# vasudeva-ram/Julia-NewtonRaphsonHANK

Hardware: AMD Instinct MI355X
Metric: sequence-space JVPs/sec (household block: BackwardIteration+ForwardIteration+aggregation, Krusell-Smith T=300) (higher is better)
Workload: dtype f64; 1 GPU; ks_2000x11_T300_N32; grid=2000x11, T=300, tangents_per_gpu=32, step=1 dual-sweep pass: primal + N tangents (hank_primal_jvp), parallelism=tangent-sharded x1

## Files before the change

julia-newtonraphsonhank_amd/csrc/hank_device.h:

```cpp
#pragma once
#include <hip/hip_runtime.h>
#include <stdint.h>
#include "hank_geom.h"

#ifndef HANK_XFWD_LQ
#define HANK_XFWD_LQ 1
#endif
#ifndef HANK_XFWD_EARLY_BATCH
#define HANK_XFWD_EARLY_BATCH 0
#endif

namespace hank {

struct Consts {
    int n_a, n_e, G, P;
    int n_hh;
    int diet;
    double beta, gamma, bc;
    const double *a, *z, *Pi;
};

struct Record {
    double *s, *kc, *A, *B, *u, *v, *pol, *lw, *ig, *Dseq;
    int *ib, *lo, *start, *clo;
    int4 *seg;
    double2 *lwg;
};

__device__ inline double wave_sum(double x) {
#pragma unroll
    for (int off = 32; off > 0; off >>= 1) x += __shfl_down(x, off, 64);
    return x;
}
__device__ inline double block_sum(double x, double *red, int nthreads) {
    const int lane = threadIdx.x & 63, wv = threadIdx.x >> 6;
    const int nw = (nthreads + 63) >> 6;
    x = wave_sum(x);
    __syncthreads();
    if (lane == 0) red[wv] = x;
    __syncthreads();
    double r = 0.0;
    if (threadIdx.x == 0)
        for (int k = 0; k < nw; k++) r += red[k];
    return r;
}

__device__ __forceinline__ void lds_barrier() { asm volatile("s_waitcnt lgkmcnt(0)\n\ts_barrier" ::: "memory"); }

__device__ __forceinline__ void st_wt(double *p, double x) {
    __hip_atomic_store(reinterpret_cast<unsigned long long *>(p), (unsigned long long)__double_as_longlong(x), __ATOMIC_RELAXED, __HIP_MEMORY_SCOPE_AGENT);
}

__device__ __forceinline__ double mix_mul(double p, double v) { return p * v; }
__device__ __forceinline__ double2 mix_mul(double p, double2 v) { return make_double2(p * v.x, p * v.y); }
__device__ __forceinline__ double mix_add(double a, double b) { return a + b; }
__device__ __forceinline__ double2 mix_add(double2 a, double2 b) { return make_double2(a.x + b.x, a.y + b.y); }
template <typename T>
__device__ __forceinline__ T mix_sum(T acc, const T *V, int vs, const double *P, int ps, int k0, int n) {
    int k = k0;
    for (; k + 3 < n; k += 4) {
        const T v0 = V[k * vs], v1 = V[(k + 1) * vs], v2 = V[(k + 2) * vs], v3 = V[(k + 3) * vs];
        const double p0 = P[k * ps], p1 = P[(k + 1) * ps], p2 = P[(k + 2) * ps], p3 = P[(k + 3) * ps];
// ... 411 lines not shown
    lds_barrier();
    if constexpr (NX > 0) {
#pragma unroll
        for (int o = 0; o < NX; o++) sh[o][e * 64 + lane] = vadd(partx[o], paggx[o]);
        lds_barrier();
        if (e == 0) {
#pragma unroll
            for (int o = 0; o < NX; o++) {
                VT s = sh[o][lane];
                for (int k = 1; k < c.n_e; k++) s = vadd(s, sh[o][k * 64 + lane]);
                for (int off = 32; off >= g.NC; off >>= 1) s = vadd(s, vshfl_xor(s, off));
                if (rl == 0 && nok) hx.parts[(((size_t)t * nbx_total + bidx) * NX + o) * N + n] = s;
            }
        }
    }
    if (e == 0) {
        VT s = red[lane], s2 = red2[lane];
        for (int k = 1; k < c.n_e; k++) { s = vadd(s, red[k * 64 + lane]); s2 = vadd(s2, red2[k * 64 + lane]); }
        for (int off = 32; off >= g.NC; off >>= 1) { s = vadd(s, vshfl_xor(s, off)); s2 = vadd(s2, vshfl_xor(s2, off)); }
        if (rl == 0 && nok) {
            aggpart[((size_t)t * nbx_total + bidx) * 2 * N + n] = s;
            aggpart[((size_t)t * nbx_total + bidx) * 2 * N + N + n] = s2;
        }
    }
}

constexpr int HX_NS = 5;

constexpr int ADJ_KS = 3;

template <typename VT>
__device__ __forceinline__ VT adj_rows_sum(VT v, int NC) {
    for (int off = 32; off >= NC; off >>= 1) v = vadd(v, vshfl_xor(v, off));
    return v;
}

template <typename VT, int NX>
struct AdjHx { const double *f, *fc; const VT *ybx; };
template <typename VT>
struct AdjHx<VT, 0> {};

struct SsCtl { int stop, iters; double resid; };

enum { ERR_KNOTS = 3, ERR_DOMAIN = 4, ERR_NONMONO = 6 };

__device__ inline void set_err(int *err, int code, int t, int e, int j) {
    if (atomicCAS(&err[0], 0, code) == 0) {
        err[1] = t;
        err[2] = e;
        err[3] = j;
    }
}

__device__ __forceinline__ void lottery_body(const Consts &c, const Record &R, int col, int *err, int write_seg, int use_ib, int *shlo, int *sh_clo, int4 *lq = nullptr) {
    const int t = col / c.n_e, e = col % c.n_e;
    const size_t base = (size_t)col * c.n_a;
    const int n = c.n_a;
    if (threadIdx.x == 0) *sh_clo = 0;
    __syncthreads();
    for (int j = threadIdx.x; j < n; j += blockDim.x) {
        const double p = R.pol[base + j];
        int lo = -1, hi = n;
        if (use_ib) {
            const int g0 = min(max(R.ib[base + j], 0), n - 2);
            const double a0 = c.a[g0], a1 = c.a[g0 + 1];
            if (a0 < p && p <= a1) { lo = g0; hi = g0 + 1; }
            else if (g0 > 0 && p <= a0 && c.a[g0 - 1] < p) { lo = g0 - 1; hi = g0; }
        }
        while (hi - lo > 1) {
            const int mid = lo + ((hi - lo) >> 1);
            if (c.a[mid] < p) lo = mid; else hi = mid;
        }
        int l;
        double w, ig;
        if (hi == 0) {
            l = 0; w = 0.0; ig = 0.0;
            atomicMax(sh_clo, j + 1);
        } else if (hi >= n) {
            l = n - 2; w = 1.0; ig = 0.0;
        } else {
            l = hi - 1;
            const double gap = c.a[hi] - c.a[l];
            w = (p - c.a[l]) / gap;
            ig = 1.0 / gap;
        }
        R.lo[base + j] = l; R.lw[base + j] = w; R.ig[base + j] = ig;
        if (lq) lq[base + j] = make_int4(__double2loint(w), __double2hiint(w), l, (hi == 0 || hi >= n) ? 1 : 0);
        shlo[j] = (hi == 0) ? -1 : l;
    }
    __syncthreads();
    const int clo = *sh_clo;
    if (threadIdx.x == 0) R.clo[col] = clo;
    int *st = R.start + (size_t)col * (n + 1);
    int *shst = shlo + n;
    for (int j = threadIdx.x; j < n; j += blockDim.x) {
        const int prev = j ? shlo[j - 1] : -1, cur = shlo[j];
        if (cur < prev) set_err(err, ERR_NONMONO, t, e, j);
        for (int r = (prev < 0 ? 0 : prev + 1); r <= cur; r++) shst[r] = j;
        if (j == n - 1)
            for (int r = (cur < 0 ? 0 : cur + 1); r <= n; r++) shst[r] = n;
    }
    __syncthreads();
    for (int r = threadIdx.x; r <= n; r += blockDim.x) st[r] = shst[r];
    if (write_seg)
        for (int r = threadIdx.x; r < n; r += blockDim.x)
            R.seg[base + r] = make_int4(r > 0 ? shst[r - 1] : shst[r], shst[r], shst[r + 1], 0);
}

struct AdjLane { int e, nl, rl, RB, m; bool mok; };
__device__ __forceinline__ AdjLane adj_lane(const AdjGeom &g) {
    AdjLane L;
    const int lane = threadIdx.x & 63;
    L.e = __builtin_amdgcn_readfirstlane((int)(threadIdx.x >> 6));
    L.nl = lane & (g.NC - 1); L.rl = lane >> g.lgNC; L.RB = 64 >> g.lgNC;
    L.m = blockIdx.y * g.NC + L.nl;
    L.mok = L.m < g.MV;
    return L;
}

template <typename VT, typename Load, typename Begin, typename Src>
__device__ __forceinline__ void adj_dist_body(const Consts &c, const Record &R, const AdjGeom &g, const AdjLane &L, int t, double *adj_sh, Load load,
                                              Begin begin, Src src) {
    const int NS = g.R + 2, n = c.n_a, ne = c.n_e;
    VT *tile = reinterpret_cast<VT *>(adj_sh);
    double *Pish = adj_sh + (size_t)ne * NS * g.NC * (sizeof(VT) / sizeof(double));
    const int e = L.e, nl = L.nl, rl = L.rl, RB = L.RB;
    const int r0 = blockIdx.x * g.R, r1 = min(r0 + g.R, n);
    for (int k = threadIdx.x; k < ne * ne; k += 64 * ne) Pish[k] = c.Pi[k];
#pragma unroll
    for (int k = 0; k < ADJ_KS; k++) {
        const int slot = rl + k * RB;
        if (slot < NS) {
            const int row = slot == g.R + 1 ? 0 : r0 + slot;
            VT v;
            vzero(v);
            if (L.mok && row <= r1 && row < n) v = load(row);
            tile[((size_t)e * NS + slot) * g.NC + nl] = v;
        }
    }
// ... 134 lines not shown
```

julia-newtonraphsonhank_amd/csrc/hank_hip.hip:

```cpp
#include "hank_kernels.h"
#include "hank_xsweep.h"
#include "hank_xspec.h"
#include "hank_jacobian.h"
#include "hank_wide.h"
#include "hank_hetx.h"
#include "hank_scen.h"
#include "hank_ssbatch.h"
#include "hank_adjoint.h"
#include "hank_boundary.h"
#include "hank_ssdiff_launch.h"
#include "../../include/hank_hip.h"

#include <cstdarg>
#include <cstdio>
#include <cstdlib>
#include <cstring>
#include <initializer_list>
#include <list>
#include <mutex>
#include <new>
#include <vector>

using namespace hank;

// ... 156 lines not shown
    void destroy() { for (One &o : s) { if (o.ev0) (void)hipEventDestroy(o.ev0); if (o.ev1) (void)hipEventDestroy(o.ev1); } }
    hipError_t begin(Span k, hipStream_t st) { s[k].valid = false; s[k].from = s[k].ev0; return hipEventRecord(s[k].ev0, st); }
    hipError_t end(Span k, hipStream_t st, int launches) { const hipError_t e = hipEventRecord(s[k].ev1, st); s[k].launches = launches; s[k].valid = e == hipSuccess; return e; }
    hipError_t end_begin(Span k, int launches, Span next, hipStream_t st) { s[next].valid = false; s[next].from = s[k].ev1; return end(k, st, launches); }
    void invalidate(std::initializer_list<Span> ks) { for (Span k : ks) s[k].valid = false; }
    void absent(Span k, int launches) { s[k].valid = false; s[k].launches = launches; }
    hipError_t read(Span k, double *ms, int32_t *launches) const {
        float f = -1.f;
        const hipError_t e = s[k].valid ? hipEventElapsedTime(&f, s[k].from, s[k].ev1) : hipSuccess;
        *ms = e == hipSuccess ? f : -1.0;
        if (launches) *launches = s[k].launches;
        return e;
    }
};
enum Stat { SWEEP_LAUNCHES, TANGENT_WORKSPACES_ALLOCATED, GRAPHS_CAPTURED, SCHEDULE, FALLBACKS, VFI_ITERATIONS, PRIMAL_MEMO_HITS, PRIMAL_SWEEPS, N_STATS };

struct hank_ctx {
    int device = 0;
    Consts c{};
    Record R{};
    int T = 0;
    DevBuf<double> d_a, d_z, d_Pi;
    DevBuf<double> d_ss_value;
    double *d_ss_D = nullptr;
    DevBuf<double> d_xhh, d_agg, d_aggpart;
    DevBuf<double> d_agg_rm;
    DevBuf<double> d_zd;
    DevBuf<int> d_err;
    int nbp = 0;
    bool boundary_set = false, primal_done = false;
    hipStream_t own_stream = nullptr, stream = nullptr;
    hipStream_t side_stream = nullptr;
    hipEvent_t ev_fork = nullptr, ev_side = nullptr;
    bool side_pending = false;
    GraphExec g_pback, g_pfwd;
    Spans spans;
    std::list<TanWork> tws;
    int schedule = 2;
    bool forced_xcd = false;
    TanBatch batch;
    int xjvp_max = 64;
    XWork xw;
    struct { DevBuf<double> dpT, iota, E, Cp, F, Dv, W, dsum; int N = 0, n_het = 0; } fn;
    int wide_mode = 0, wide_min = 80, num_cus = 256, wide_r = 2;
    size_t lds_max = 65536;
    DevBuf<char> rec_slab;
    size_t rec_bytes = 0;
    int4 *rec_lq = nullptr;
    double *rec_iga = nullptr;
    DevBuf<int> d_ibw;
    bool seg_valid = true;
    bool lwg_valid = true;
    long long lwg_builds = 0;
    bool wprep_valid = false;
    std::list<WTan> wtans;
    std::list<CotWork> cws;
    CotBatch cot;
    DevBuf<int> d_adj_sb;
    bool adj_seg_valid = false;
    DevBuf<double> d_bnd_q;
    HxRecord hx;
    ScenWork scen;
    int scen_pending = 0;
    std::vector<double> h_Pi, h_z;
    long long stats[N_STATS] = {};
    bool memo_on = true;
    bool xdual_back = true;
    bool memo_valid = false;
    std::vector<double> memo_xhh;
    int n_het = 2;
    DevBuf<char> hx_slab;
    size_t hx_bytes = 0;
    bool stationary = false;
    std::vector<double> h_ss_value, h_ss_D;
    hipEvent_t ev_stream = nullptr;
    char errmsg[512] = {0};
};

static int fail(hank_ctx *ctx, int code, const char *fmt, ...);
static int het_max(const hank_ctx *ctx) { return ctx->c.n_hh > 2 ? 4 : 3; }
static int hx_count(const hank_ctx *ctx) { return het_max(ctx) - 2; }
static void batch_none(hank_ctx *ctx) { ctx->batch.current = false; ctx->batch.ws = nullptr; }
static void cot_none(hank_ctx *ctx) { ctx->cot = CotBatch(); }
static void cot_ran(hank_ctx *ctx, const void *ws, int M, const double *pbar) { ctx->cot = CotBatch{true, M, ws, pbar}; }
static void batch_ran(hank_ctx *ctx, int family, const void *ws, int N, const double *dagg_cm, const double *dpol, const std::vector<XPass> *passes = nullptr) {
    ctx->batch = TanBatch{family, true, N, ws, dagg_cm, dpol, passes};
}
static void batch_ran_boundary(hank_ctx *ctx, const void *ws, int N, const double *dagg_cm, const double *dpol, const double *zm) {
    batch_ran(ctx, 0, ws, N, dagg_cm, dpol);
    ctx->batch.boundary = true;
    ctx->batch.bnd_zm = zm;
}
static int batch_current(hank_ctx *ctx, int N, const TanBatch **out) {
    if (!ctx->batch.current || ctx->batch.N != N) return fail(ctx, HANK_ERR_NOT_READY, "no tangent sweep with N=%d is current", N);
    *out = &ctx->batch;
    return HANK_OK;
}
static void record_rewritten(hank_ctx *ctx, bool seg_written, bool lwg_written) {
    ctx->primal_done = true; ctx->seg_valid = seg_written; ctx->lwg_valid = lwg_written;
    ctx->wprep_valid = false; ctx->xw.src_valid = false; ctx->xw.rng_valid = false; ctx->adj_seg_valid = false; ctx->hx.valid = false;
    batch_none(ctx);
    cot_none(ctx);
}
static void record_gone(hank_ctx *ctx) {
    record_rewritten(ctx, false, false);
    ctx->primal_done = false;
}
static hipError_t join_side(hank_ctx *ctx) {
    if (!ctx->side_pending) return hipSuccess;
    ctx->side_pending = false;
    return hipStreamWaitEvent(ctx->stream, ctx->ev_side, 0);
}

static int fail(hank_ctx *ctx, int code, const char *fmt, ...) {
    if (ctx) {
        va_list ap;
        va_start(ap, fmt);
        vsnprintf(ctx->errmsg, sizeof(ctx->errmsg), fmt, ap);
        va_end(ap);
    }
    return code;
}

static int het_count_ok(hank_ctx *ctx, const char *who, int n_het, bool declared, bool rest_ok = true) {
    const int max_het = het_max(ctx);
    if (n_het < 1 || n_het > max_het || !rest_ok)
        return fail(ctx, HANK_ERR_BAD_ARG, "%s: bad argument: n_het must be 1..%d (the policy variable, consumption, Value%s), got %d", who, max_het, max_het > 3 ? ", UCE" : "", n_het);
    if (declared && n_het > ctx->n_het)
        return fail(ctx, HANK_ERR_NOT_READY, "%s: %d outputs asked for, %d declared: call hank_set_het_outputs first", who, n_het, ctx->n_het);
    return HANK_OK;
}

static int hip_status(hipError_t e) {
    if (e == hipErrorOutOfMemory) return HANK_ERR_NOMEM;
    if (e == hipErrorNoDevice || e == hipErrorInvalidDevice || e == hipErrorNotInitialized || e == hipErrorInsufficientDriver) return HANK_ERR_NO_DEVICE;
    return HANK_ERR_LAUNCH;
}
#define HIPC(ctx, call)                                                                         \
    do {                                                                                        \
        hipError_t e_ = (call);                                                                 \
        if (e_ != hipSuccess)                                                                   \
            return fail(ctx, hip_status(e_),                                                   \
                        "HIP error %d (%s) at %s:%d: %s", (int)e_, hipGetErrorString(e_),       \
                        __FILE__, __LINE__, #call);                                             \
    } while (0)

struct DeviceGuard {
    int prev = -1;
    bool switched = false, ok = true;
    explicit DeviceGuard(const hank_ctx *ctx);
    ~DeviceGuard() { if (switched) (void)hipSetDevice(prev); }
};
DeviceGuard::DeviceGuard(const hank_ctx *ctx) {
    if (!ctx) return;
    if (hipGetDevice(&prev) != hipSuccess) { ok = false; return; }
    if (prev != ctx->device) { switched = hipSetDevice(ctx->device) == hipSuccess; ok = switched; }
}
#define ENTER(ctx)                                                                                                       \
// ... 450 lines not shown
        w.passes.push_back(ps);
    }
    if ((int)w.passes.size() > XPASS_MAX) return fail(ctx, HANK_ERR_BAD_ARG, "N=%d needs %d passes, at most %d per call", N, (int)w.passes.size(), XPASS_MAX);
    HIPC(ctx, w.dxhh.alloc((size_t)c.n_hh * P * N));
    HIPC(ctx, w.dxr.alloc(P * N)); HIPC(ctx, w.dxw.alloc(P * N)); HIPC(ctx, w.dxt.alloc(P * N));
    HIPC(ctx, w.dpol.alloc(off));
    const size_t W = (size_t)XG * X.dmax, nb = (size_t)X.Sact;
    HIPC(ctx, w.daggpart.alloc(2 * P * nb * W));
    HIPC(ctx, hipMemsetAsync(w.daggpart, 0, sizeof(double) * 2 * P * nb * W, ctx->stream));
    HIPC(ctx, w.dagg_pass.alloc(2 * P * W));
    HIPC(ctx, w.dagg_cm.alloc(2 * P * N));
    return HANK_OK;
}
static int x_ensure_tan(hank_ctx *ctx, int N, XTan **out) {
    const int nmax = 8 * ctx->xw.dmax * XPASS_MAX;
    if (N > nmax) return fail(ctx, HANK_ERR_BAD_ARG, "N=%d exceeds %d directions per call", N, nmax);
    return tan_cache_get(ctx, ctx->xw.tans, N, [ctx](XTan &w) { return x_build_tan(ctx, w); }, out);
}

static dim3 x_block(const XWork &X, const Consts &c) {
    const bool fits = 64 * (c.n_e + 1) <= X.maxt && X.syncwave;
    return dim3(fits ? 64 * (c.n_e + 1) : 64 * c.n_e);
}

template <typename F>
static void x_by_maxt(const XWork &X, F launch) { if (X.maxt == 768) launch(std::integral_constant<int, 768>()); else launch(std::integral_constant<int, 1024>()); }
#define XL(...) hipLaunchKernelGGL((__VA_ARGS__), dim3(X.grid), x_block(X, c), lds, sec.stream(), a)
static bool x_has_dual_back(const XWork &X) { return X.maxt == 768; }
static void x_launch_dual_back(XSection &sec, XWork &X, const Consts &c, int D, const XDualBackArgs &a) {
    const size_t lds = x_lds_dual_back(c, D);
    if (!x_has_dual_back(X)) return;
    const XSpec sp = x_spec(X.xspec, c.n_e, c.gamma, c.diet);
    X.inst[0] = sp.ne; X.inst[1] = sp.crra;
    if (!sp.ne && !sp.crra) {
        if (D == 1) XL(k_xdual_back<1, 768>);
        else if (D == 2) XL(k_xdual_back<2, 768>);
        else XL(k_xdual_back<4, 768>);
        return;
    }
    auto by_d = [&](auto ne, auto crra) {
        constexpr int NE = decltype(ne)::value, CRRA = decltype(crra)::value;
        if (D == 1) XL(k_xdual_back<1, 768, NE, CRRA>);
        else if (D == 2) XL(k_xdual_back<2, 768, NE, CRRA>);
        else XL(k_xdual_back<4, 768, NE, CRRA>);
    };
    auto by_crra = [&](auto ne) {
        if (sp.crra) by_d(ne, std::integral_constant<int, 1>()); else if constexpr (decltype(ne)::value != 0) by_d(ne, std::integral_constant<int, 0>());
    };
    if (sp.ne == 4) by_crra(std::integral_constant<int, 4>());
    else if (sp.ne == 7) by_crra(std::integral_constant<int, 7>());
    else if (sp.ne == 11) by_crra(std::integral_constant<int, 11>());
    else by_crra(std::integral_constant<int, 0>());
}
static void x_launch_fwd(XSection &sec, XWork &X, const Consts &c, int D, bool val, const XSweepFwdArgs &a) {
    if (val && D > 0) { X.inst[2] = 0; X.inst[3] = 0; }
#if HANK_XFWD_LQ
    if (val && D > 0 && x_lds_fwd_lq(c, D) <= (size_t)X.lds_max) {
        const size_t lds = x_lds_fwd_lq(c, D);
        x_by_maxt(X, [&](auto mt) {
            constexpr int MT = decltype(mt)::value;
            if (D == 1) XL(k_xfwd<1, true, MT, true>);
            else if (D == 2) XL(k_xfwd<2, true, MT, true>);
            else if (D == 4) { if constexpr (MT == 768) XL(k_xfwd<4, true, MT, true>); }
        });
        return;
    }
#endif
    const size_t lds = x_lds_fwd(c, D, val || D == 0);
    x_by_maxt(X, [&](auto mt) {
        constexpr int MT = decltype(mt)::value;
        if (D == 0) XL(k_xfwd<0, true, MT>);
        else if (D == 1) { if (val) XL(k_xfwd<1, true, MT>); else XL(k_xfwd<1, false, MT>); }
        else if (D == 2) { if (val) XL(k_xfwd<2, true, MT>); else XL(k_xfwd<2, false, MT>); }
        else if (D == 4) { if constexpr (MT == 768) { if (val) XL(k_xfwd<4, true, MT>); else XL(k_xfwd<4, false, MT>); } }
    });
}
static void x_launch_primal_back(XSection &sec, const XWork &X, const Consts &c, const XBackArgs &a) { const size_t lds = x_lds_primal_back(c); x_by_maxt(X, [&](auto mt) { XL(k_xprimal_back<decltype(mt)::value>); }); }
static void x_launch_tan_back(XSection &sec, const XWork &X, const Consts &c, int D, const XTanBackArgs &a) {
    const size_t lds = x_lds_tan_back(c, D);
    x_by_maxt(X, [&](auto mt) {
        constexpr int MT = decltype(mt)::value;
        if (D == 1) XL(k_xtan_back<1, MT>);
        else if (D == 2) XL(k_xtan_back<2, MT>);
        else if (D == 4) { if constexpr (MT == 768) XL(k_xtan_back<4, MT>); }
    });
}
static void x_ensure_rng(XSection &sec) {
    hank_ctx *ctx = sec.ctx;
    XWork &X = ctx->xw;
    if (X.rng_valid) return;
    hipLaunchKernelGGL(k_xunits_fwd, dim3((unsigned)ctx->c.P, (unsigned)X.Sact), dim3(256), 0, sec.stream(), ctx->c, ctx->R, X.Sact, X.srcF, X.unitsF, X.unit_overflow, X.ucap);
    X.rng_valid = true;
}

static int ensure_seg(hank_ctx *ctx) {
    if (ctx->seg_valid) return HANK_OK;
    hipLaunchKernelGGL(k_seg_build, dim3((unsigned)(ctx->c.P * ctx->c.n_e)), dim3(256), 0, ctx->stream, ctx->c, ctx->R, ctx->c.P * ctx->c.n_e);
    HIPC(ctx, hipGetLastError());
    ctx->seg_valid = true;
    return HANK_OK;
}
static int ensure_lwg(hank_ctx *ctx) {
    if (ctx->lwg_valid) return HANK_OK;
    const XWork &X = ctx->xw;
    hipLaunchKernelGGL(k_xlwg_build, dim3((unsigned)(ctx->c.P * ctx->c.n_e)), dim3(256), 0, ctx->stream, ctx->c, ctx->R, X.Dvirt, X.D0own, X.Sact);
    HIPC(ctx, hipGetLastError());
    ctx->lwg_valid = true;
    ctx->lwg_builds++;
    return HANK_OK;
}
static int x_sync_reset(XSection &sec, XSync *base, int count, int where) {
    hank_ctx *ctx = sec.ctx;
    HIPC(ctx, hipMemsetAsync(base, 0, sizeof(XSync) * (size_t)count, sec.stream()));
    if (ctx->xw.fault && ctx->xw.fault != 3 && (ctx->xw.fault_where & where)) hipLaunchKernelGGL(k_xpoison, dim3(1), dim3(64), 0, sec.stream(), base, count, (unsigned)ctx->xw.fault);
    return HANK_OK;
}

static void x_rho(XSection &sec) {
    hank_ctx *ctx = sec.ctx;
    hipLaunchKernelGGL(k_xrho, dim3((unsigned)((ctx->c.P + 255) / 256)), dim3(256), 0, sec.stream(), ctx->d_xhh, ctx->c.n_hh, ctx->c.P, ctx->xw.rho);
}
static void x_tan_in(XSection &sec, XTan *w) {
    const Consts &c = sec.ctx->c;
    hipLaunchKernelGGL(k_tan_in, dim3((unsigned)(((size_t)c.P * w->N + 255) / 256)), dim3(256), 0, sec.stream(), w->dxhh, c.n_hh, c.P, w->N, w->dxr, w->dxw, w->dxt);
}
static int x_tan_front(XSection &sec, XTan *w) {
    hank_ctx *ctx = sec.ctx; XWork &X = ctx->xw;
    const int rc = x_sync_reset(sec, X.sync + 2, 2 * (int)w->passes.size(), 2); if (rc) return rc;
    x_tan_in(sec, w);
    x_rho(sec);
    if (!X.src_valid) {
        hipLaunchKernelGGL(k_xsrc_back, dim3((unsigned)ctx->c.P, X.Sact), dim3(256), 0, sec.stream(), ctx->c, ctx->R, X.Sact, X.srcB);
        X.src_valid = true;
    }
    return HANK_OK;
}
static XRecOff x_rec_off(const hank_ctx *ctx) {
    const Record &R = ctx->R;
    const char *b = ctx->rec_slab;
    auto off = [&](const void *p) { return (unsigned)((const char *)p - b); };
    XRecOff o{};
    o.rec = b; o.bytes = (unsigned)ctx->rec_bytes;
    o.pol = off(R.pol); o.ib = off(R.ib); o.A = off(R.A); o.B = off(R.B); o.u = off(R.u); o.v = off(R.v); o.s = off(R.s); o.kc = off(R.kc);
    o.lo = off(R.lo); o.lw = off(R.lw); o.ig = off(R.ig); o.Dseq = off(R.Dseq);
    o.lq = ctx->rec_lq ? off(ctx->rec_lq) : 0u;
    return o;
}
static bool x_dual_addr_fits(const hank_ctx *ctx) {
    const Consts &c = ctx->c;
    return x_addr_fits(ctx->rec_bytes, (unsigned long long)c.P, XG, (unsigned long long)c.G, XD_MAX, (unsigned long long)((c.n_a + XRW - 1) / XRW), XUCAP);
}
static int x_back(XSection &sec, XTan *dual = nullptr) {
    hank_ctx *ctx = sec.ctx; XWork &X = ctx->xw;
    const Consts &c = ctx->c;
    XBackArgs ab{};
    ab.c = c; ab.ss_value = ctx->d_ss_value; ab.xhh = ctx->d_xhh; ab.rho = X.rho; ab.sy = X.sync; ab.st_s = X.st_s;
// ... 16 lines not shown
#if HANK_XFWD_LQ
    if (lq) {
        hipLaunchKernelGGL(k_lottery_lq, dim3((unsigned)(c.P * c.n_e)), dim3(256), sizeof(int) * (2 * (size_t)c.n_a + 2), sec.stream(), c, ctx->R, c.P * c.n_e, ctx->d_err, seg ? 1 : 0, 1, ctx->rec_lq);
        return;
    }
#endif
    hipLaunchKernelGGL(k_lottery, dim3((unsigned)(c.P * c.n_e)), dim3(256), sizeof(int) * (2 * (size_t)c.n_a + 2), sec.stream(), c, ctx->R, c.P * c.n_e, ctx->d_err, seg ? 1 : 0, 1);
}
static int x_tan_back(XSection &sec, XTan *w) {
    hank_ctx *ctx = sec.ctx; XWork &X = ctx->xw;
    const int np = (int)w->passes.size();
    XTanBackArgs ab{};
    ab.c = ctx->c; ab.R = ctx->R; ab.rho = X.rho; ab.xhh = ctx->d_xhh; ab.dxr = w->dxr; ab.dxw = w->dxw; ab.dxt = w->dxt; ab.Ntot = w->N; ab.st_ds = X.st_ds;
    ab.src = X.neigh ? X.srcB.get() : nullptr;
    ab.stall = X.fault == 3 ? 1 : 0;
    HIPC(ctx, ctx->spans.begin(TAN_BACK, sec.stream()));
    for (int p = 0; p < np; p++) {
        const XPass &ps = w->passes[p];
        ab.n0 = ps.n0; ab.N = ps.N; ab.groups = ps.groups; ab.sy = X.sync + 2 + 2 * p; ab.dpol = w->dpol + ps.dpol_off;
        x_launch_tan_back(sec, X, ctx->c, ps.D, ab);
    }
    HIPC(ctx, ctx->spans.end(TAN_BACK, sec.stream(), np));
    return HANK_OK;
}
static void x_value_epilogue(XSection &sec) {
    hank_ctx *ctx = sec.ctx; const XWork &X = ctx->xw;
    const Consts &c = ctx->c;
    const size_t P = c.P;
    hipStream_t s = sec.stream();
    hipLaunchKernelGGL(k_reduce_parts, dim3((unsigned)P, 1), dim3(256), 0, s, X.aggpart, X.Sact, 2, ctx->d_agg_rm);
    hipLaunchKernelGGL(k_tan_out, dim3((unsigned)((2 * P + 255) / 256)), dim3(256), 0, s, ctx->d_agg_rm, (int)P, 2, ctx->d_agg);
    hipLaunchKernelGGL(k_xfix_D, dim3((unsigned)((P * c.n_e + 255) / 256)), dim3(256), 0, s, c, ctx->R.Dseq, X.Dvirt, X.Sact, X.D0own);
}
static XSweepFwdArgs x_fwd_args(const hank_ctx *ctx, bool val) {
    const XWork &X = ctx->xw;
    XSweepFwdArgs fa{};
    fa.c = ctx->c; fa.R = ctx->R; fa.src = X.srcF; fa.units = X.unitsF; fa.overflow = X.unit_overflow; fa.all_members = X.neigh ? 0 : 1;
    if (val) { fa.D0 = ctx->d_ss_D; fa.Dvirt = X.Dvirt; fa.aggpart = X.aggpart; }
    return fa;
}
static int x_fwd_value(XSection &sec) {
    hank_ctx *ctx = sec.ctx; XWork &X = ctx->xw;
    XSweepFwdArgs fa = x_fwd_args(ctx, true);
    fa.sy = X.sync + 1; fa.st = X.st_D; fa.groups = 1;
    HIPC(ctx, ctx->spans.begin(PRIMAL_FWD, sec.stream()));
    x_launch_fwd(sec, X, ctx->c, 0, true, fa);
    HIPC(ctx, ctx->spans.end(PRIMAL_FWD, sec.stream(), 1));
    x_value_epilogue(sec);
    return HANK_OK;
}
static int x_tan_fwd(XSection &sec, XTan *w, int p, bool val) {
    hank_ctx *ctx = sec.ctx; XWork &X = ctx->xw;
    const XPass &ps = w->passes[p];
    if (!val) { const int rc = ensure_lwg(ctx); if (rc) return rc; }
    XSweepFwdArgs fa = x_fwd_args(ctx, val);
    fa.sy = X.sync + 2 + 2 * p + 1; fa.st = X.st_dD; fa.daggpart = w->daggpart; fa.groups = ps.groups; fa.dpol = w->dpol + ps.dpol_off;
    fa.ro = x_rec_off(ctx); fa.dpol_bytes = (unsigned)((size_t)ctx->c.P * ps.groups * ctx->c.G * ps.D * sizeof(double));
    fa.iga = ctx->rec_iga ? (unsigned)((const char *)ctx->rec_iga - (const char *)ctx->rec_slab) : 0u;
    x_launch_fwd(sec, X, ctx->c, ps.D, val, fa);
    return HANK_OK;
}
static void x_tan_reduce(XSection &sec, XTan *w, int p) {
    hank_ctx *ctx = sec.ctx;
    const size_t P = ctx->c.P;
    const XPass &ps = w->passes[p];
    const int W = XG * ps.D;
    hipStream_t s = sec.stream();
    hipLaunchKernelGGL(k_reduce_parts, dim3((unsigned)P, (2 * W + 63) / 64), dim3(256), 0, s, w->daggpart, ctx->xw.Sact, 2 * W, w->dagg_pass);
    hipLaunchKernelGGL(k_xout, dim3((unsigned)((P * ps.N + 255) / 256)), dim3(256), 0, s, w->dagg_pass, (int)P, 2 * W, 0, ps.n0, ps.N, w->dagg_cm);
    hipLaunchKernelGGL(k_xout, dim3((unsigned)((P * ps.N + 255) / 256)), dim3(256), 0, s, w->dagg_pass, (int)P, 2 * W, W, ps.n0, ps.N, w->dagg_cm + P * (size_t)w->N);
}
static int x_tan_fwd_from(XSection &sec, XTan *w, int first) {
    hank_ctx *ctx = sec.ctx;
    const int np = (int)w->passes.size();
    for (int p = first; p < np; p++) {
        const int rc = x_tan_fwd(sec, w, p, false); if (rc) return rc;
        if (p == np - 1) HIPC(ctx, ctx->spans.end(TAN_FWD, sec.stream(), np));
        x_tan_reduce(sec, w, p);
    }
    return HANK_OK;
}
static void x_dual_epilogue(XSection &sec, XTan *w, double *d_agg_out, double *d_dagg_out) {
    hank_ctx *ctx = sec.ctx; const XWork &X = ctx->xw;
    const Consts &c = ctx->c;
    const XPass &ps = w->passes[0];
    const int W = XG * ps.D, per = 2 * W + 2 + c.n_e;
    hipLaunchKernelGGL(k_xdual_epilogue, dim3((unsigned)(((size_t)c.P * per + 255) / 256)), dim3(256), 0, sec.stream(), c, X.aggpart, w->daggpart, X.Sact, W, ps.n0, ps.N, w->N,
                       ctx->d_agg_rm, ctx->d_agg, w->dagg_pass, w->dagg_cm, ctx->R.Dseq, X.Dvirt, X.D0own, d_agg_out, d_dagg_out);
}

static int x_status(hank_ctx *ctx, const char *what, const XSync *fetched) {
    XWork &X = ctx->xw;
    std::vector<XSync> own;
    if (!fetched) {
        if (!X.ready || X.last_blocks == 0) return HANK_OK;
        int uo = 0;
        HIPC(ctx, hipMemcpy(&uo, X.unit_overflow, sizeof(int), hipMemcpyDeviceToHost));
        if (uo) {
            HIPC(ctx, hipMemsetAsync(X.unit_overflow, 0, sizeof(int), ctx->stream));
            return fail(ctx, HANK_ERR_SWEEP, "persistent forward sweep: a member's walk over its sources needs more than %d work units (a savings policy this flat is served by the per-period launches)", XUCAP);
        }
        own.resize((size_t)X.last_blocks);
        HIPC(ctx, hipMemcpy(own.data(), X.sync, sizeof(XSync) * own.size(), hipMemcpyDeviceToHost));
    }
    const XSync *h = fetched ? fetched : own.data();
    for (size_t k = 0; k < (fetched ? 1 : own.size()); k++)
// ... 328 lines not shown
        return HANK_OK;
    }
    HIPC(ctx, join_side(ctx));
    HIPC(ctx, hipMemcpyAsync(ctx->d_ss_value, ss_end_value, sizeof(double) * G, hipMemcpyHostToDevice, ctx->stream));
    HIPC(ctx, hipMemcpyAsync(ctx->d_ss_D, ss_init_D, sizeof(double) * G, hipMemcpyHostToDevice, ctx->stream));
    {
        const int ne = ctx->c.n_e, na = ctx->c.n_a, P = ctx->c.P;
        std::vector<double> m(ne, 0.0), m2(ne), zd(2 * (size_t)P);
        for (int e = 0; e < ne; e++) for (int i = 0; i < na; i++) m[e] += ss_init_D[(size_t)e * na + i];
        for (int t = 0; t < P; t++) {
            for (int e2 = 0; e2 < ne; e2++) { double v = 0.0; for (int e = 0; e < ne; e++) v += ctx->h_Pi[e + (size_t)ne * e2] * m[e]; m2[e2] = v; }
            m.swap(m2);
            double z = 0.0, one = 0.0;
            for (int e = 0; e < ne; e++) { z += ctx->h_z[e] * m[e]; one += m[e]; }
            zd[t] = z; zd[(size_t)P + t] = one;
        }
        HIPC(ctx, hipMemcpyAsync(ctx->d_zd, zd.data(), sizeof(double) * 2 * P, hipMemcpyHostToDevice, ctx->stream));
    }
    HIPC(ctx, hipStreamSynchronize(ctx->stream));
    ctx->boundary_set = true;
    record_gone(ctx);
    ctx->memo_valid = false;
    ctx->stationary = false;
    ctx->h_ss_value.assign(ss_end_value, ss_end_value + G);
    ctx->h_ss_D.assign(ss_init_D, ss_init_D + G);
    ctx->errmsg[0] = 0;
    return HANK_OK;
}

static void note_primal_x(hank_ctx *ctx, const double *xhh) {
    const size_t n = (size_t)ctx->c.n_hh * ctx->c.P, nh = ctx->c.n_hh;
    if (!xhh) { ctx->memo_valid = false; ctx->stationary = false; return; }
    ctx->memo_xhh.assign(xhh, xhh + n);
    ctx->memo_valid = true;
    bool constant = true;
    for (size_t k = nh; k < n && constant; k++) constant = xhh[k] == xhh[k - nh];
    ctx->stationary = constant;
}

static int run_primal(hank_ctx *ctx, double *d_agg_out) {
    HIPC(ctx, join_side(ctx));
    HIPC(ctx, ctx->spans.begin(PRIMAL_BACK, ctx->stream));
    HIPC(ctx, hipGraphLaunch(ctx->g_pback, ctx->stream));
    HIPC(ctx, ctx->spans.end(PRIMAL_BACK, ctx->stream, ctx->c.P + 2));
    HIPC(ctx, hipEventRecord(ctx->ev_fork, ctx->stream));
    HIPC(ctx, hipStreamWaitEvent(ctx->side_stream, ctx->ev_fork, 0));
    HIPC(ctx, ctx->spans.begin(PRIMAL_FWD, ctx->side_stream));
    HIPC(ctx, hipGraphLaunch(ctx->g_pfwd, ctx->side_stream));
    HIPC(ctx, ctx->spans.end(PRIMAL_FWD, ctx->side_stream, ctx->c.P + 1));
    HIPC(ctx, copy_agg(ctx, d_agg_out, hipMemcpyDeviceToDevice, ctx->side_stream));
    HIPC(ctx, hipEventRecord(ctx->ev_side, ctx->side_stream));
    ctx->side_pending = true;
    ctx->spans.invalidate({DUAL_BACK, DUAL_FWD});
    record_rewritten(ctx, true, true);
    return HANK_OK;
}

static int x_primal(hank_ctx *ctx, const double *xhh, hipMemcpyKind kind, double *d_agg_out) {
    int rc = x_setup(ctx); if (rc) return rc;
    HIPC(ctx, hipMemcpyAsync(ctx->d_xhh, xhh, sizeof(double) * ctx->c.n_hh * ctx->c.P, kind, ctx->stream));
    XSection sec(ctx);
    HIPC(ctx, sec.opened());
    rc = x_sync_reset(sec, ctx->xw.sync, 2, 1); if (rc) return rc;
    zero_err(ctx, sec.stream());
    x_rho(sec);
    rc = x_back(sec); if (rc) return rc;
    x_lottery(sec, true);
    record_rewritten(ctx, true, true);
    x_ensure_rng(sec);
    rc = x_fwd_value(sec); if (rc) return rc;
    HIPC(ctx, hipGetLastError());
    HIPC(ctx, sec.close());
    ctx->stats[SWEEP_LAUNCHES] += 2;
    ctx->xw.last_blocks = 2;
    ctx->spans.invalidate({TAN_BACK, TAN_FWD, DUAL_BACK, DUAL_FWD});
    HIPC(ctx, copy_agg(ctx, d_agg_out, hipMemcpyDeviceToDevice, ctx->stream));
    return HANK_OK;
}
static int x_jvp(hank_ctx *ctx, const double *dxhh, hipMemcpyKind kind, int N, double *d_dagg_out) {
    int rc = x_setup(ctx); if (rc) return rc;
    XTan *w = nullptr;
    rc = x_ensure_tan(ctx, N, &w); if (rc) return rc;
    const int np = (int)w->passes.size();
    HIPC(ctx, hipMemcpyAsync(w->dxhh, dxhh, sizeof(double) * ctx->c.n_hh * ctx->c.P * N, kind, ctx->stream));
    XSection sec(ctx);
    HIPC(ctx, sec.opened());
    rc = x_tan_front(sec, w); if (rc) return rc;
    x_ensure_rng(sec);
    rc = x_tan_back(sec, w); if (rc) return rc;
    HIPC(ctx, ctx->spans.begin(TAN_FWD, sec.stream()));
    rc = x_tan_fwd_from(sec, w, 0); if (rc) return rc;
    HIPC(ctx, hipGetLastError());
    HIPC(ctx, sec.close());
    ctx->stats[SWEEP_LAUNCHES] += 2 * np;
    ctx->xw.last_blocks = 2 + 2 * np;
    ctx->spans.invalidate({DUAL_BACK, DUAL_FWD});
    batch_ran(ctx, 1, w, N, w->dagg_cm, w->dpol, &w->passes);
    HIPC(ctx, copy_dagg(ctx, d_dagg_out, w->dagg_cm, N, hipMemcpyDeviceToDevice));
    return HANK_OK;
}
static void x_dual_ran(hank_ctx *ctx, XTan *w, int launches) {
    ctx->stats[SWEEP_LAUNCHES] += launches;
    ctx->xw.last_blocks = 2 + 2 * (int)w->passes.size();
    ctx->spans.absent(PRIMAL_FWD, 1);
    ctx->spans.invalidate({DUAL_BACK, DUAL_FWD});
    batch_ran(ctx, 1, w, w->N, w->dagg_cm, w->dpol, &w->passes);
}
static int x_dual_two(hank_ctx *ctx, XTan *w, const double *xhh, const double *dxhh, hipMemcpyKind kind, double *d_agg_out, double *d_dagg_out) {
    const size_t nP = (size_t)ctx->c.n_hh * ctx->c.P;
    const int np = (int)w->passes.size();
    XSection sec(ctx);
    HIPC(ctx, sec.opened());
    HIPC(ctx, hipMemcpyAsync(w->dxhh, dxhh, sizeof(double) * nP * w->N, kind, sec.stream()));
    HIPC(ctx, hipMemcpyAsync(ctx->d_xhh, xhh, sizeof(double) * nP, kind, sec.stream()));
    int rc = x_sync_reset(sec, ctx->xw.sync, 2, 1); if (rc) return rc;
    zero_err(ctx, sec.stream());
    x_rho(sec);
    rc = x_back(sec); if (rc) return rc;
    x_lottery(sec, true, true);
    record_rewritten(ctx, true, false);
    x_ensure_rng(sec);
    rc = x_tan_front(sec, w);
    if (!rc) rc = x_tan_back(sec, w);
    if (rc) return rc;
    HIPC(ctx, ctx->spans.begin(TAN_FWD, sec.stream()));
    rc = x_tan_fwd(sec, w, 0, true); if (rc) return rc;
    if (np == 1) {
        HIPC(ctx, ctx->spans.end(TAN_FWD, sec.stream(), 1));
        x_dual_epilogue(sec, w, d_agg_out, d_dagg_out);
    } else {
        x_value_epilogue(sec);
        x_tan_reduce(sec, w, 0);
        rc = x_tan_fwd_from(sec, w, 1); if (rc) return rc;
    }
    HIPC(ctx, hipGetLastError());
    HIPC(ctx, sec.close());
    x_dual_ran(ctx, w, 1 + 2 * np);
    if (np > 1) {
        HIPC(ctx, copy_agg(ctx, d_agg_out, hipMemcpyDeviceToDevice, ctx->stream));
        HIPC(ctx, copy_dagg(ctx, d_dagg_out, w->dagg_cm, w->N, hipMemcpyDeviceToDevice));
    }
    return HANK_OK;
}
static int x_dual_fused(hank_ctx *ctx, XTan *w, const double *xhh, const double *dxhh, hipMemcpyKind kind, bool prologue, double *d_agg_out, double *d_dagg_out) {
    XWork &X = ctx->xw;
    const size_t nP = (size_t)ctx->c.n_hh * ctx->c.P;
    XSection sec(ctx);
    HIPC(ctx, sec.opened());
    if (prologue) {
        hipLaunchKernelGGL(k_xdual_prologue, dim3(64), dim3(256), 0, sec.stream(), xhh, ctx->d_xhh, dxhh, w->dxhh, ctx->c.n_hh, ctx->c.P, w->N, X.rho, w->dxr, w->dxw, w->dxt,
                           reinterpret_cast<xv4u *>(X.sync.get()), sizeof(XSync) * 4 / sizeof(xv4u), ctx->d_err);
    } else {
        HIPC(ctx, hipMemcpyAsync(w->dxhh, dxhh, sizeof(double) * nP * w->N, kind, sec.stream()));
        HIPC(ctx, hipMemcpyAsync(ctx->d_xhh, xhh, sizeof(double) * nP, kind, sec.stream()));
        int rc = x_sync_reset(sec, X.sync, 2, 1);
        if (!rc) rc = x_sync_reset(sec, X.sync + 2, 2, 2);
        if (rc) return rc;
        zero_err(ctx, sec.stream());
        x_rho(sec);
        x_tan_in(sec, w);
    }
    int rc = x_back(sec, w); if (rc) return rc;
    x_lottery(sec, false, true);
    record_rewritten(ctx, false, false);
    x_ensure_rng(sec);
    HIPC(ctx, ctx->spans.begin(TAN_BACK, sec.stream()));
    HIPC(ctx, ctx->spans.end(TAN_BACK, sec.stream(), 1));
    HIPC(ctx, ctx->spans.begin(TAN_FWD, sec.stream()));
    rc = x_tan_fwd(sec, w, 0, true); if (rc) return rc;
    HIPC(ctx, ctx->spans.end(TAN_FWD, sec.stream(), 1));
    x_dual_epilogue(sec, w, d_agg_out, d_dagg_out);
    HIPC(ctx, hipGetLastError());
    HIPC(ctx, sec.close());
    x_dual_ran(ctx, w, 2);
    return HANK_OK;
}
static bool x_dual_back_fits(const hank_ctx *ctx, int D);
static int x_dual(hank_ctx *ctx, const double *xhh, const double *dxhh, hipMemcpyKind kind, int N, double *d_agg_out, double *d_dagg_out) {
    int rc = x_setup(ctx); if (rc) return rc;
    XTan *w = nullptr;
    rc = x_ensure_tan(ctx, N, &w); if (rc) return rc;
    if (w->passes.size() != 1 || !x_dual_back_fits(ctx, w->passes[0].D)) return x_dual_two(ctx, w, xhh, dxhh, kind, d_agg_out, d_dagg_out);
    return x_dual_fused(ctx, w, xhh, dxhh, kind, kind == hipMemcpyDeviceToDevice && !ctx->xw.fault, d_agg_out, d_dagg_out);
}
static bool use_x_primal(const hank_ctx *ctx) { return ctx->schedule >= 1; }
static bool x_tan_fits(const hank_ctx *ctx, int N) {
    const XWork &X = ctx->xw;
    int D = 1;
    while (XG * D < N && D < X.dmax) D *= 2;
    return std::max(x_lds_tan_back(ctx->c, D), x_lds_fwd(ctx->c, D, true)) <= (size_t)X.lds_max;
}
static bool use_x_jvp(const hank_ctx *ctx, int N) { return (ctx->schedule == 1 || (ctx->schedule == 2 && N <= ctx->xjvp_max)) && x_tan_fits(ctx, N); }
static bool x_dual_back_fits(const hank_ctx *ctx, int D) {
    const XWork &X = ctx->xw;
    return ctx->xdual_back && x_has_dual_back(X) && 64 * (ctx->c.n_e + 1) <= X.maxt && x_lds_dual_back(ctx->c, D) <= (size_t)X.lds_max;
}
static bool use_x_fused(const hank_ctx *ctx, int N) {
    if (ctx->schedule < 1 || !x_tan_fits(ctx, N) || !x_dual_addr_fits(ctx)) return false;
    if (ctx->schedule == 1) return true;
    return N <= XG * ctx->xw.dmax && x_dual_back_fits(ctx, ctx->xw.dmax);
}

static int check_rates(hank_ctx *ctx, const double *xhh) {
    for (int t = 0; t < ctx->c.P; t++)
        if (!(1.0 + xhh[ctx->c.n_hh * t] > 0.0)) return fail(ctx, HANK_ERR_DOMAIN, "1 + r must be positive (period %zu)", (size_t)t + 1);
    return HANK_OK;
}
static int enqueue_primal(hank_ctx *ctx, const double *xhh, hipMemcpyKind kind, double *d_agg_out) {
    if (use_x_primal(ctx)) return x_primal(ctx, xhh, kind, d_agg_out);
    HIPC(ctx, hipMemcpyAsync(ctx->d_xhh, xhh, sizeof(double) * ctx->c.n_hh * ctx->c.P, kind, ctx->stream));
    return run_primal(ctx, d_agg_out);
}

int hank_primal_dev(hank_ctx *ctx, const double *d_xhh, double *d_agg_out) {
    ENTER(ctx);
    if (!ctx || !d_xhh) return fail(ctx, HANK_ERR_BAD_ARG, "null pointer");
    if (!ctx->boundary_set) return fail(ctx, HANK_ERR_NOT_READY, "hank_set_boundary must be called first");
    note_primal_x(ctx, nullptr);
    ctx->stats[PRIMAL_SWEEPS]++;
    return enqueue_primal(ctx, d_xhh, hipMemcpyDeviceToDevice, d_agg_out);
}

int hank_check(hank_ctx *ctx) {
    ENTER(ctx);
    if (!ctx) return HANK_ERR_BAD_ARG;
    bool moved = false;
    const int rc = fallback_decision(ctx, device_verdict(ctx, THE_RECORD), &moved);
    return rc ? rc : scen_pending_verdict(ctx);
}

int hank_primal(hank_ctx *ctx, const double *xhh, double *agg_out) {
    ENTER(ctx);
    if (!ctx || !xhh) return fail(ctx, HANK_ERR_BAD_ARG, "null pointer");
    if (!ctx->boundary_set) return fail(ctx, HANK_ERR_NOT_READY, "hank_set_boundary must be called first");
    { const int rrc = check_rates(ctx, xhh); if (rrc) return rrc; }
    note_primal_x(ctx, nullptr);
    const int rc = run_settled(ctx, [&] { return enqueue_primal(ctx, xhh, hipMemcpyHostToDevice, nullptr); });
    if (rc) return rc;
    if (agg_out) {
        HIPC(ctx, copy_agg(ctx, agg_out, hipMemcpyDeviceToHost, ctx->stream));
        HIPC(ctx, hipStreamSynchronize(ctx->stream));
    }
    note_primal_x(ctx, xhh);
    ctx->stats[PRIMAL_SWEEPS]++;
    ctx->errmsg[0] = 0;
    return HANK_OK;
}

static int run_jvp(hank_ctx *ctx, TanWork &w, bool bnd, bool zm, int NX) {
    const int grc = ensure_tan_graphs(ctx, w, bnd, NX);
    if (grc) return grc;
    HIPC(ctx, ctx->spans.begin(TAN_BACK, ctx->stream));
    HIPC(ctx, hipGraphLaunch(w.tan_back(bnd), ctx->stream));
    HIPC(ctx, ctx->spans.end(TAN_BACK, ctx->stream, ctx->c.P + (bnd ? 4 : 2)));
    HIPC(ctx, join_side(ctx));
    { const int src = ensure_seg(ctx); if (src) return src; }
    { const int src = ensure_lwg(ctx); if (src) return src; }
    HIPC(ctx, ctx->spans.begin(TAN_FWD, ctx->stream));
    HIPC(ctx, hipGraphLaunch(w.tan_fwd(bnd, NX), ctx->stream));
    HIPC(ctx, ctx->spans.end(TAN_FWD, ctx->stream, ctx->c.P + (bnd ? 5 : 3) + (NX > 0 ? 1 : 0)));
    if (bnd) batch_ran_boundary(ctx, &w, w.N, w.dagg_cm, w.dpol, zm ? w.bnd_zm.get() : nullptr);
    else batch_ran(ctx, 0, &w, w.N, w.dagg_cm, w.dpol);
    return HANK_OK;
}

struct TanReq {
    int n_het;
    const double *dxhh, *dvalue_end, *dD_init;
    hipMemcpyKind kind;
    bool seeded;
};
static int ensure_bnd_bufs(hank_ctx *ctx, TanWork &w);
static int ensure_hx_record(hank_ctx *ctx);

static int enqueue_tan_launch(hank_ctx *ctx, const TanReq &q, int N, TanWork **out) {
    const Consts &c = ctx->c;
    const size_t P = c.P, GN = (size_t)c.G * N;
    const int NX = q.n_het > 2 ? q.n_het - 2 : 0, SX = hx_count(ctx);
    TanWork *w = nullptr;
    int rc = ensure_tanwork(ctx, N, &w);
    if (rc) return rc;
    if (q.seeded && (rc = ensure_bnd_bufs(ctx, *w)) != HANK_OK) return rc;
    if (q.n_het > 0 && !w->het_out) HIPC(ctx, w->het_out.alloc(P * het_max(ctx) * N));
    if (NX > 0) {
        HIPC(ctx, join_side(ctx));
        rc = ensure_hx_record(ctx);
        if (rc) return rc;
        if (!w->hx_T) {
            HIPC(ctx, w->hx_parts.alloc(P * (size_t)w->nbf * SX * N));
            HIPC(ctx, w->hx_T.alloc((size_t)N * P * SX));
        }
    }
    const struct { double *dst; const double *src; size_t count; } in[3] = {{w->dxhh, q.dxhh, c.n_hh * P * N}, {w->bnd_dV, q.dvalue_end, GN}, {w->bnd_dD, q.dD_init, GN}};
    for (int k = 0; k < (q.seeded ? 3 : 1); k++) {
        if (in[k].src) HIPC(ctx, hipMemcpyAsync(in[k].dst, in[k].src, sizeof(double) * in[k].count, q.kind, ctx->stream));
        else HIPC(ctx, hipMemsetAsync(in[k].dst, 0, sizeof(double) * in[k].count, ctx->stream));
    }
    rc = run_jvp(ctx, *w, q.seeded, q.dD_init != nullptr, NX);
    if (rc) return rc;
    *out = w;
    return HANK_OK;
}
static int enqueue_tan_raw(hank_ctx *ctx, const TanReq &q, int N, double *d_dagg_out) {
    TanWork *w = nullptr;
    const int rc = enqueue_tan_launch(ctx, q, N, &w);
    if (rc) return rc;
    HIPC(ctx, copy_dagg(ctx, d_dagg_out, w->dagg_cm, N, hipMemcpyDeviceToDevice));
    return HANK_OK;
// ... 54 lines not shown
        for (int e = 0; e < ne; e++) {
            double a = 0.0, b = 0.0;
            for (int e2 = 0; e2 < ne; e2++) { a += ctx->h_Pi[e + (size_t)ne * e2] * q[e2]; b += ctx->h_Pi[e + (size_t)ne * e2] * o[e2]; }
            q2[e] = a; o2[e] = b;
        }
        q.swap(q2); o.swap(o2);
        for (int e = 0; e < ne; e++) { Q[(size_t)t * ne + e] = q[e]; Q[((size_t)P + t) * ne + e] = o[e]; }
    }
    DevBuf<double> buf;
    HIPC(ctx, buf.alloc(Q.size()));
    HIPC(ctx, hipMemcpyAsync(buf, Q.data(), sizeof(double) * Q.size(), hipMemcpyHostToDevice, ctx->stream));
    HIPC(ctx, hipStreamSynchronize(ctx->stream));
    ctx->d_bnd_q = std::move(buf);
    return HANK_OK;
}
static int ensure_bnd_bufs(hank_ctx *ctx, TanWork &w) {
    const size_t P = ctx->c.P, GN = (size_t)ctx->c.G * w.N;
    const int rc = ensure_bnd_q(ctx);
    if (rc) return rc;
    if (!w.bnd_zm) {
        HIPC(ctx, w.bnd_dV.alloc(GN));
        HIPC(ctx, w.bnd_dD.alloc(GN));
        HIPC(ctx, w.bnd_m0.alloc((size_t)w.N * ctx->c.n_e));
        HIPC(ctx, w.bnd_zm.alloc(2 * P * w.N));
    }
    return HANK_OK;
}
int hank_jvp_boundary_dev(hank_ctx *ctx, const double *d_dxhh, const double *d_dvalue_end, const double *d_dD_init, int32_t N, double *d_dagg_out) {
    ENTER(ctx);
    const TanReq q{0, d_dxhh, d_dvalue_end, d_dD_init, hipMemcpyDeviceToDevice, true};
    const int rc = tan_seed_args(ctx, "hank_jvp_boundary", false, q, N, d_dagg_out, false);
    return rc ? rc : enqueue_tan_raw(ctx, q, N, d_dagg_out);
}

int hank_jvp_boundary(hank_ctx *ctx, const double *dxhh, const double *dvalue_end, const double *dD_init, int32_t N, double *dagg_out) {
    ENTER(ctx);
    const TanReq q{0, dxhh, dvalue_end, dD_init, hipMemcpyHostToDevice, true};
    int rc = tan_seed_args(ctx, "hank_jvp_boundary", false, q, N, dagg_out, true);
    if (!rc) rc = enqueue_tan_raw(ctx, q, N, nullptr);
    if (rc) return rc;
    return tan_host_tail(ctx, dagg_out, ctx->batch.dagg_cm, (size_t)ctx->c.P * N);
}

static int run_fused(hank_ctx *ctx, TanWork &w) {
    const int grc = ensure_dual_graphs(ctx, w);
    if (grc) return grc;
    HIPC(ctx, join_side(ctx));
    HIPC(ctx, ctx->spans.begin(DUAL_BACK, ctx->stream));
    HIPC(ctx, hipGraphLaunch(w.g_fback, ctx->stream));
    HIPC(ctx, ctx->spans.end_begin(DUAL_BACK, ctx->c.P + 5, DUAL_FWD, ctx->stream));
    HIPC(ctx, hipGraphLaunch(w.g_ffwd, ctx->stream));
    HIPC(ctx, ctx->spans.end(DUAL_FWD, ctx->stream, ctx->c.P + 5));
    ctx->spans.invalidate({PRIMAL_BACK, PRIMAL_FWD, TAN_BACK, TAN_FWD});
    record_rewritten(ctx, true, true);
    batch_ran(ctx, 0, &w, w.N, w.dagg_cm, w.dpol);
    return HANK_OK;
}

static int enqueue_primal_jvp(hank_ctx *ctx, const double *xhh, const double *dxhh, hipMemcpyKind kind, int N, double *d_agg_out, double *d_dagg_out) {
    if (use_x_fused(ctx, N)) return x_dual(ctx, xhh, dxhh, kind, N, d_agg_out, d_dagg_out);
    TanWork *w = nullptr;
    int rc = ensure_tanwork(ctx, N, &w);
    if (rc) return rc;
    const size_t P = ctx->c.P;
    HIPC(ctx, join_side(ctx));
    HIPC(ctx, hipMemcpyAsync(ctx->d_xhh, xhh, sizeof(double) * ctx->c.n_hh * P, kind, ctx->stream));
    HIPC(ctx, hipMemcpyAsync(w->dxhh, dxhh, sizeof(double) * ctx->c.n_hh * P * N, kind, ctx->stream));
    rc = run_fused(ctx, *w);
    if (rc) return rc;
    HIPC(ctx, copy_agg(ctx, d_agg_out, hipMemcpyDeviceToDevice, ctx->stream));
    HIPC(ctx, copy_dagg(ctx, d_dagg_out, w->dagg_cm, N, hipMemcpyDeviceToDevice));
    return HANK_OK;
}

int hank_primal_jvp_dev(hank_ctx *ctx, const double *d_xhh, const double *d_dxhh, int32_t N, double *d_agg_out,
                        double *d_dagg_out) {
    ENTER(ctx);
    if (!ctx || !d_xhh || !d_dxhh || N < 1) return fail(ctx, HANK_ERR_BAD_ARG, "bad argument (N=%d)", N);
    if (!ctx->boundary_set) return fail(ctx, HANK_ERR_NOT_READY, "hank_set_boundary must be called first");
    if (use_wide(ctx, N)) {
        const int rc = hank_primal_dev(ctx, d_xhh, d_agg_out);
        return rc ? rc : hank_jvp_dev(ctx, d_dxhh, N, d_dagg_out);
    }
    note_primal_x(ctx, nullptr);
    ctx->stats[PRIMAL_SWEEPS]++;
    return enqueue_primal_jvp(ctx, d_xhh, d_dxhh, hipMemcpyDeviceToDevice, N, d_agg_out, d_dagg_out);
}

int hank_primal_jvp(hank_ctx *ctx, const double *xhh, const double *dxhh, int32_t N, double *agg_out, double *dagg_out) {
    ENTER(ctx);
    if (!ctx || !xhh || !dxhh || !dagg_out || N < 1) return fail(ctx, HANK_ERR_BAD_ARG, "bad argument (N=%d)", N);
    if (!ctx->boundary_set) return fail(ctx, HANK_ERR_NOT_READY, "hank_set_boundary must be called first");
    const size_t P = ctx->c.P;
    int rc = check_rates(ctx, xhh);
    if (rc) return rc;
    if (ctx->memo_on && ctx->primal_done && ctx->memo_valid && ctx->memo_xhh.size() == (size_t)ctx->c.n_hh * P &&
        memcmp(ctx->memo_xhh.data(), xhh, sizeof(double) * ctx->c.n_hh * P) == 0) {
        ctx->stats[PRIMAL_MEMO_HITS]++;
        rc = hank_jvp(ctx, dxhh, N, dagg_out);
        if (rc) return rc;
        if (agg_out) {
            HIPC(ctx, join_side(ctx));
            HIPC(ctx, copy_agg(ctx, agg_out, hipMemcpyDeviceToHost, ctx->stream));
            HIPC(ctx, hipStreamSynchronize(ctx->stream));
        }
        return HANK_OK;
    }
// ... 11 lines not shown
    ctx->stats[PRIMAL_SWEEPS]++;
    ctx->errmsg[0] = 0;
    return HANK_OK;
}

static int ensure_fn(hank_ctx *ctx, int n_het) {
    if (ctx->fn.n_het >= n_het) return HANK_OK;
    const size_t P = ctx->c.P, G = ctx->c.G, NP = P * ctx->c.n_hh, S = 16, nh = n_het;
    if (ctx->fn.dpT) HIPC(ctx, hipStreamSynchronize(ctx->stream));
    ctx->fn = {};
    auto alloc = [&]() -> int {
        HIPC(ctx, ctx->fn.dpT.alloc(G * NP)); HIPC(ctx, ctx->fn.iota.alloc(G * NP));
        HIPC(ctx, ctx->fn.E.alloc(nh * P * G)); HIPC(ctx, ctx->fn.Cp.alloc(S * nh * P * NP));
        HIPC(ctx, ctx->fn.F.alloc(nh * P * NP)); HIPC(ctx, ctx->fn.Dv.alloc(nh * NP));
        HIPC(ctx, ctx->fn.W.alloc(nh * G)); HIPC(ctx, ctx->fn.dsum.alloc(nh * ctx->c.n_hh));
        return HANK_OK;
    };
    const int rc = alloc();
    if (rc) {
        ctx->fn = {};
        (void)hipGetLastError();
        return rc;
    }
    ctx->fn.n_het = n_het;
    return HANK_OK;
}

static int stationary_record(hank_ctx *ctx, const char *name) {
    if (!ctx->primal_done) return fail(ctx, HANK_ERR_NOT_READY, "hank_primal must be called before %s", name);
    if (!ctx->stationary)
        return fail(ctx, HANK_ERR_NOT_READY, "%s needs the recorded primal to be hank_primal at a CONSTANT path (the steady state; SteadyStateJacobian.jl:53-57): "
                    "the last primal was recorded at a path that varies over time, or through a device-pointer entry", name);
    const int P = ctx->c.P, G = ctx->c.G;
    hipStream_t s = ctx->stream;
    std::vector<double> p0((size_t)G), p1((size_t)G);
    HIPC(ctx, join_side(ctx));
    HIPC(ctx, hipMemcpyAsync(p0.data(), ctx->R.pol, sizeof(double) * G, hipMemcpyDeviceToHost, s));
    HIPC(ctx, hipMemcpyAsync(p1.data(), ctx->R.pol + (size_t)(P - 1) * G, sizeof(double) * G, hipMemcpyDeviceToHost, s));
    HIPC(ctx, hipStreamSynchronize(s));
    double scale = 0.0, diff = 0.0;
    for (int k = 0; k < G; k++) { scale = std::max(scale, fabs(p1[k])); diff = std::max(diff, fabs(p0[k] - p1[k])); }
    if (!(diff <= 1e-6 * std::max(scale, 1e-300)))
        return fail(ctx, HANK_ERR_NOT_READY, "%s: the recorded primal is not stationary (policy of period 1 and of period %d differ by %.3g): "
                    "it needs hank_primal at the steady state with the steady state as both boundaries", name, P, diff);
    return HANK_OK;
}

static int fake_news(hank_ctx *ctx, int n_het, double *F_out, double *Dv_out) {
    const char *name = n_het ? "hank_fake_news_het" : "hank_fake_news";
    { const int nrc = stationary_record(ctx, name); if (nrc) return nrc; }
    const Consts &c = ctx->c;
    const int P = c.P, G = c.G, N = c.n_hh, NP = P * N, S = 16, nh = n_het ? n_het : 1;
    hipStream_t s = ctx->stream;
    { const int src = ensure_seg(ctx); if (src) return src; }
    { const int src = ensure_lwg(ctx); if (src) return src; }
    TanWork *wp = nullptr;
    int rc = ensure_tanwork(ctx, N, &wp);
    if (rc) return rc;
    TanWork &w = *wp;
    rc = ensure_tan_graphs(ctx, w, false, 0);
    if (rc) return rc;
    rc = ensure_fn(ctx, nh);
    if (rc) return rc;
    HIPC(ctx, join_side(ctx));
    hipLaunchKernelGGL(k_fn_seed, dim3((unsigned)((N * P * N + 255) / 256)), dim3(256), 0, s, w.dxhh, N, P);
    HIPC(ctx, hipGraphLaunch(w.tan_back(false), s));
    batch_none(ctx);
    hipLaunchKernelGGL(k_fn_transpose, dim3((unsigned)((G + 31) / 32), (unsigned)((P + 31) / 32), (unsigned)N), dim3(256), 0, s, w.dpol, P, G, N, ctx->fn.dpT);
    hipLaunchKernelGGL(k_fn_impulse, dim3((unsigned)c.n_a, (unsigned)((NP + 255) / 256)), dim3(256), 0, s, c, ctx->R, ctx->fn.dpT, NP, ctx->fn.iota);
    const size_t PG = (size_t)P * G;
    const double *Wd = ctx->R.Dseq + G;
    if (n_het) {
        hipLaunchKernelGGL(k_fn_het_record, dim3((unsigned)nh), dim3(256), 0, s, c, ctx->R, ctx->d_xhh, PG, ctx->fn.E, ctx->fn.W, ctx->fn.dsum);
        for (int u = 0; u + 1 < P; u++)
            hipLaunchKernelGGL(k_fn_expect_het, dim3((unsigned)((G + 255) / 256), (unsigned)nh), dim3(256), 0, s, c, ctx->R, ctx->fn.E, PG, u);
        Wd = ctx->fn.W;
    } else {
        HIPC(ctx, hipMemcpyAsync(ctx->fn.E, ctx->R.pol, sizeof(double) * G, hipMemcpyDeviceToDevice, s));
        for (int u = 0; u + 1 < P; u++)
            hipLaunchKernelGGL(k_fn_expect, dim3((unsigned)((G + 255) / 256)), dim3(256), 0, s, c, ctx->R, ctx->fn.E + (size_t)u * G, ctx->fn.E + (size_t)(u + 1) * G);
    }
    const int kchunk = ((G + S - 1) / S + 15) / 16 * 16, MP = nh * P;
    hipLaunchKernelGGL(k_fn_gemm, dim3((unsigned)((NP + 63) / 64), (unsigned)((MP + 63) / 64), (unsigned)S), dim3(256), 0, s, ctx->fn.E, ctx->fn.iota, ctx->fn.Cp, MP, NP, G, kchunk);
    hipLaunchKernelGGL(k_fn_reduce, dim3((unsigned)(((size_t)MP * NP + 255) / 256)), dim3(256), 0, s, ctx->fn.Cp, MP * NP, S, ctx->fn.F);
    hipLaunchKernelGGL(k_fn_gemm, dim3((unsigned)((NP + 63) / 64), (unsigned)((nh + 63) / 64), (unsigned)S), dim3(256), 0, s, Wd, ctx->fn.dpT, ctx->fn.Cp, nh, NP, G, kchunk);
    hipLaunchKernelGGL(k_fn_reduce, dim3((unsigned)((nh * NP + 255) / 256)), dim3(256), 0, s, ctx->fn.Cp, nh * NP, S, ctx->fn.Dv);
    HIPC(ctx, hipGetLastError());
    std::vector<double> hF((size_t)MP * NP), hD((size_t)nh * NP), hd((size_t)nh * N, 0.0);
    HIPC(ctx, hipMemcpyAsync(hF.data(), ctx->fn.F, sizeof(double) * hF.size(), hipMemcpyDeviceToHost, s));
    HIPC(ctx, hipMemcpyAsync(hD.data(), ctx->fn.Dv, sizeof(double) * hD.size(), hipMemcpyDeviceToHost, s));
    if (n_het) HIPC(ctx, hipMemcpyAsync(hd.data(), ctx->fn.dsum, sizeof(double) * hd.size(), hipMemcpyDeviceToHost, s));
    HIPC(ctx, hipStreamSynchronize(s));
    rc = device_verdict(ctx, THE_RECORD);
    if (rc) return rc;
    for (int o = 0; o < nh; o++)
        for (int k = 0; k < N; k++)
            for (int t = 0; t < P; t++) {
                const int j = P - 1 - t;
                const size_t ko = (size_t)k + (size_t)N * o;
                const double dv = hD[(size_t)o * NP + (size_t)t * N + k];
                Dv_out[j + (size_t)P * ko] = (o > 0 && j == 0) ? dv + hd[ko] : dv;
                for (int u = 0; u < P; u++) F_out[u + (size_t)P * (j + (size_t)P * ko)] = hF[((size_t)o * P + u) * NP + (size_t)t * N + k];
            }
    ctx->errmsg[0] = 0;
    return HANK_OK;
}
// ... 50 lines not shown
        double *dst = d_out + P * col;
        col += (size_t)N_k[k];
        if (bytes == 0) continue;
        ENTER(ck);
        if (ck->device == c0->device) {
            HIPC(c0, hipMemcpyAsync(dst, d_blocks[k], bytes, hipMemcpyDeviceToDevice, ck->stream));
        } else {
            const hipError_t pe = hipDeviceEnablePeerAccess(c0->device, 0);
            if (pe != hipSuccess && pe != hipErrorPeerAccessAlreadyEnabled) { (void)hipGetLastError(); return fail(c0, HANK_ERR_NO_DEVICE, "no peer access from device %d to device %d (%s)", ck->device, c0->device, hipGetErrorString(pe)); }
            (void)hipGetLastError();
            HIPC(c0, hipMemcpyPeerAsync(dst, c0->device, d_blocks[k], ck->device, bytes, ck->stream));
        }
        if (ck != c0 && ck->stream != c0->stream) {
            HIPC(c0, hipEventRecord(ck->ev_stream, ck->stream));
            HIPC(c0, hipStreamWaitEvent(c0->stream, ck->ev_stream, 0));
        }
    }
    c0->errmsg[0] = 0;
    return HANK_OK;
}

int hank_info(hank_ctx *ctx, int64_t out[8]) {
    if (!ctx || !out) return HANK_ERR_BAD_ARG;
    out[0] = ctx->batch.family; out[1] = ctx->wide_mode; out[2] = ctx->wide_min; out[3] = w_supported(ctx) ? 1 : 0;
    out[4] = ctx->xjvp_max; out[5] = ctx->c.diet; out[6] = (int64_t)ctx->rec_bytes; out[7] = ctx->lwg_builds;
    return HANK_OK;
}

int hank_last_timings(hank_ctx *ctx, double *out_ms, int32_t *launches) {
    if (!ctx || !out_ms) return HANK_ERR_BAD_ARG;
    ENTER(ctx);
    HIPC(ctx, join_side(ctx));
    HIPC(ctx, hipStreamSynchronize(ctx->stream));
    for (int k = PRIMAL_BACK; k <= DUAL_FWD; k++) HIPC(ctx, ctx->spans.read((Span)k, &out_ms[k], launches ? &launches[k] : nullptr));
    return HANK_OK;
}

int hank_get_policy_seq(hank_ctx *ctx, double *out) {
    if (!ctx || !out) return HANK_ERR_BAD_ARG;
    ENTER(ctx);
    if (!ctx->primal_done) return fail(ctx, HANK_ERR_NOT_READY, "no primal sweep has been run");
    HIPC(ctx, join_side(ctx));
    HIPC(ctx, hipMemcpyAsync(out, ctx->R.pol, sizeof(double) * (size_t)ctx->c.P * ctx->c.G, hipMemcpyDeviceToHost, ctx->stream));
    HIPC(ctx, hipStreamSynchronize(ctx->stream));
    return HANK_OK;
}

int hank_get_lottery_record(hank_ctx *ctx, int32_t *lo, double *lw, double *ig, void *lq, double *iga) {
    if (!ctx) return HANK_ERR_BAD_ARG;
    ENTER(ctx);
    if (!ctx->primal_done) return fail(ctx, HANK_ERR_NOT_READY, "no primal sweep has been run");
    if ((lq || iga) && !ctx->rec_lq) return fail(ctx, HANK_ERR_BAD_ARG, "hank_get_lottery_record: this build keeps no packed lottery record");
    HIPC(ctx, join_side(ctx));
    const size_t n = (size_t)ctx->c.P * ctx->c.G;
    if (lo) HIPC(ctx, hipMemcpyAsync(lo, ctx->R.lo, sizeof(int) * n, hipMemcpyDeviceToHost, ctx->stream));
    if (lw) HIPC(ctx, hipMemcpyAsync(lw, ctx->R.lw, sizeof(double) * n, hipMemcpyDeviceToHost, ctx->stream));
    if (ig) HIPC(ctx, hipMemcpyAsync(ig, ctx->R.ig, sizeof(double) * n, hipMemcpyDeviceToHost, ctx->stream));
    if (lq) HIPC(ctx, hipMemcpyAsync(lq, ctx->rec_lq, sizeof(int4) * n, hipMemcpyDeviceToHost, ctx->stream));
    if (iga) HIPC(ctx, hipMemcpyAsync(iga, ctx->rec_iga, sizeof(double) * (size_t)ctx->c.n_a, hipMemcpyDeviceToHost, ctx->stream));
    HIPC(ctx, hipStreamSynchronize(ctx->stream));
    return HANK_OK;
}

int hank_get_dist_seq(hank_ctx *ctx, double *out) {
    if (!ctx || !out) return HANK_ERR_BAD_ARG;
    ENTER(ctx);
    if (!ctx->primal_done) return fail(ctx, HANK_ERR_NOT_READY, "no primal sweep has been run");
    HIPC(ctx, join_side(ctx));
    HIPC(ctx, hipMemcpyAsync(out, ctx->R.Dseq + ctx->c.G, sizeof(double) * (size_t)ctx->c.P * ctx->c.G, hipMemcpyDeviceToHost, ctx->stream));
    HIPC(ctx, hipStreamSynchronize(ctx->stream));
    return HANK_OK;
}

static int grid_aggregates(hank_ctx *ctx, double *agg2_out, int32_t N, double *dagg2_out, bool dev) {
    if (!ctx || (!agg2_out && !dagg2_out) || N < 0) return HANK_ERR_BAD_ARG;
    ENTER(ctx);
    const hipMemcpyKind kind = dev ? hipMemcpyDeviceToDevice : hipMemcpyDeviceToHost;
    if (agg2_out) {
        if (!ctx->primal_done) return fail(ctx, HANK_ERR_NOT_READY, "no primal sweep has been run");
        HIPC(ctx, join_side(ctx));
        HIPC(ctx, copy_agg(ctx, agg2_out, kind, ctx->stream, 1));
    }
    if (dagg2_out && N > 0) {
        const TanBatch *b = nullptr;
        const int rc = batch_current(ctx, N, &b);
        if (rc) return rc;
        HIPC(ctx, copy_dagg(ctx, dagg2_out, b->dagg_cm, N, kind, 1));
    }
    if (!dev) HIPC(ctx, hipStreamSynchronize(ctx->stream));
    return HANK_OK;
}
int hank_get_grid_aggregates(hank_ctx *ctx, double *agg2_out, int32_t N, double *dagg2_out) { return grid_aggregates(ctx, agg2_out, N, dagg2_out, false); }
int hank_get_grid_aggregates_dev(hank_ctx *ctx, double *d_agg2_out, int32_t N, double *d_dagg2_out) { return grid_aggregates(ctx, d_agg2_out, N, d_dagg2_out, true); }

int hank_get_dpolicy_seq(hank_ctx *ctx, int32_t N, double *out) {
    if (!ctx || !out) return HANK_ERR_BAD_ARG;
    ENTER(ctx);
    const TanBatch *b = nullptr;
    int rc = batch_current(ctx, N, &b);
    if (rc) return rc;
    const size_t total = (size_t)ctx->c.P * ctx->c.G * N;
    DevBuf<double> tmp;
    HIPC(ctx, tmp.alloc(total));
    rc = export_dpol_dev(ctx, *b, tmp);
    if (rc) return rc;
    HIPC(ctx, hipMemcpyAsync(out, tmp, sizeof(double) * total, hipMemcpyDeviceToHost, ctx->stream));
// ... 65 lines not shown
    for (int t = 0; t < P; t++) {
        hipLaunchKernelGGL((k_adj_egm<VT>), grd, blk, ldsB, s, c, ctx->R, w.g, t, t == 0 ? 1 : 0, t == P - 1 ? 1 : 0, ctx->d_adj_sb, st[cur], st[cur ^ 1], pbar,
                           reinterpret_cast<VT *>(w.partS.get()), reinterpret_cast<VT *>(w.partM.get()));
        cur ^= 1;
    }
    hipLaunchKernelGGL(k_adj_out, dim3((unsigned)((P * w.N + 255) / 256)), dim3(256), 0, s, P, c.n_hh, w.N, w.g.nb, ctx->d_xhh, w.partS, w.partM, w.yb1,
                       ctx->d_agg + P, ctx->d_zd, w.xbar);
    return end_capture(ctx, &w.g_B);
}

static int ensure_adj_seg(hank_ctx *ctx) {
    const Consts &c = ctx->c;
    if (ctx->adj_seg_valid) return HANK_OK;
    hipLaunchKernelGGL(k_adj_seg, dim3((unsigned)(c.P * c.n_e)), dim3(256), sizeof(int) * ((size_t)c.n_a + 1), ctx->stream, c, ctx->R, c.P * c.n_e, ctx->d_adj_sb);
    HIPC(ctx, hipGetLastError());
    ctx->adj_seg_valid = true;
    return HANK_OK;
}

static int ensure_hx_record(hank_ctx *ctx) {
    const Consts &c = ctx->c;
    HxRecord &h = ctx->hx;
    if (h.valid) return HANK_OK;
    const size_t P = c.P, SX = hx_count(ctx);
    if (!h.S) {
        HIPC(ctx, h.f.alloc(SX * P * c.G));
        HIPC(ctx, h.fc.alloc(SX * P * c.G));
        HIPC(ctx, h.S.alloc(P * SX * HX_NS));
    }
    hipLaunchKernelGGL(k_hx_record, dim3((unsigned)P, (unsigned)SX), dim3(256), 0, ctx->stream, c, ctx->R, ctx->d_xhh, (int)SX, h.f.get(), h.fc.get(), h.S.get());
    HIPC(ctx, hipGetLastError());
    h.valid = true;
    return HANK_OK;
}

static int enqueue_vjp(hank_ctx *ctx, int n_het, const double *agg_bar, hipMemcpyKind kind, int M, double *d_xhh_bar, CotWork **out,
                       double *d_vend_bar = nullptr, double *d_D0_bar = nullptr) {
    const Consts &c = ctx->c;
    const size_t P = c.P;
    const int NX = n_het > 2 ? n_het - 2 : 0;
    CotWork *w = nullptr;
    int rc = tan_cache_get(ctx, ctx->cws, M, [ctx](CotWork &cw) { return build_cotwork(ctx, cw); }, &w);
    if (rc) return rc;
    if (adj_lds_dist(c, w->g, w->V) > ctx->lds_max || adj_lds_egm(c, w->g, w->V) > ctx->lds_max)
        return fail(ctx, HANK_ERR_BAD_ARG, "hank_vjp: n_e=%d needs more LDS per workgroup than the device has", c.n_e);
    if (!w->g_A) {
        if (!ctx->d_adj_sb) HIPC(ctx, ctx->d_adj_sb.alloc(P * c.n_e * ((size_t)c.n_a + 1)));
        rc = w->V == 2 ? capture_cot_graphs<double2>(ctx, *w) : capture_cot_graphs<double>(ctx, *w);
        if (rc) return rc;
    }
    hipStream_t s = ctx->stream;
    HIPC(ctx, hipMemcpyAsync(w->ybar, agg_bar, sizeof(double) * P * n_het * M, kind, s));
    HIPC(ctx, join_side(ctx));
    rc = ensure_adj_seg(ctx);
    if (rc) return rc;
    if (NX > 0) {
        rc = ensure_hx_record(ctx);
        if (rc) return rc;
        if (!w->g_AX[NX - 1]) {
            if (NX == 1) rc = w->V == 2 ? capture_cot_graph_ax<double2, 1>(ctx, *w) : capture_cot_graph_ax<double, 1>(ctx, *w);
            else rc = w->V == 2 ? capture_cot_graph_ax<double2, 2>(ctx, *w) : capture_cot_graph_ax<double, 2>(ctx, *w);
            if (rc) return rc;
        }
    }
    hipLaunchKernelGGL(k_adj_in, dim3((unsigned)((P * M + 255) / 256)), dim3(256), 0, s, w->ybar, (int)P, n_het, M, w->yb0, w->yb1);
    if (NX > 0) hipLaunchKernelGGL(k_adj_in_hx, dim3((unsigned)((P * NX * M + 255) / 256)), dim3(256), 0, s, w->ybar, (int)P, n_het, M, w->ybx.get());
    HIPC(ctx, ctx->spans.begin(VJP_A, s));
    HIPC(ctx, hipGraphLaunch(NX > 0 ? w->g_AX[NX - 1] : w->g_A, s));
    HIPC(ctx, ctx->spans.end_begin(VJP_A, (int)P, VJP_B, s));
    const dim3 tblk(BND_T, 8), tgrd((unsigned)((c.n_a + BND_T - 1) / BND_T), (unsigned)((M + BND_T - 1) / BND_T), (unsigned)c.n_e);
    if (d_D0_bar) hipLaunchKernelGGL(k_bnd_out, tgrd, tblk, 0, s, w->st[P & 1].get(), c.n_a, c.n_e, M, d_D0_bar);
    HIPC(ctx, hipGraphLaunch(w->g_B, s));
    if (d_vend_bar) {
        hipLaunchKernelGGL(k_bnd_vend, dim3((unsigned)(((size_t)c.n_a * M + 255) / 256)), dim3(256), 0, s, c, ctx->R, (int)P - 1, P == 1 ? 1 : 0, ctx->d_adj_sb.get(),
                           w->st[(P - 1) & 1].get(), w->pbar.get(), (size_t)M, w->st[P & 1].get());
        hipLaunchKernelGGL(k_bnd_out, tgrd, tblk, 0, s, w->st[P & 1].get(), c.n_a, c.n_e, M, d_vend_bar);
    }
    HIPC(ctx, hipGetLastError());
    HIPC(ctx, ctx->spans.end(VJP_B, s, (int)P + 1 + (d_D0_bar ? 1 : 0) + (d_vend_bar ? 2 : 0)));
    if (NX > 0) {
        hipLaunchKernelGGL(k_adj_hx_out, dim3((unsigned)((P * M + 255) / 256)), dim3(256), 0, s, (int)P, c.n_hh, M, NX, hx_count(ctx), w->ybx.get(),
                           ctx->hx.S.get(), w->xbar.get());
        HIPC(ctx, hipGetLastError());
    }
    cot_ran(ctx, w, M, w->pbar);
    if (d_xhh_bar) HIPC(ctx, hipMemcpyAsync(d_xhh_bar, w->xbar, sizeof(double) * c.n_hh * P * M, hipMemcpyDeviceToDevice, s));
    *out = w;
    return HANK_OK;
}
static int vjp_args(hank_ctx *ctx, int n_het, const void *in, int M, const void *out) {
    if (!ctx || !in || !out || M < 1) return fail(ctx, HANK_ERR_BAD_ARG, "hank_vjp: bad argument (M=%d)", M);
    if (n_het > 2 && n_het <= het_max(ctx))
        return fail(ctx, HANK_ERR_BAD_ARG, "hank_vjp: n_het=%d reaches Value / UCE, which are not affine in the policy: their cotangents are not implemented (n_het must be 1 or 2)", n_het);
    if (n_het < 1 || n_het > 2) return fail(ctx, HANK_ERR_BAD_ARG, "hank_vjp: n_het must be 1 (the policy variable) or 2 (and consumption), got %d", n_het);
    if (!ctx->primal_done) return fail(ctx, HANK_ERR_NOT_READY, "hank_primal must be called before hank_vjp");
    return HANK_OK;
}

static int vjp_het_args(hank_ctx *ctx, int n_het, const void *in, int M, const void *out) {
    if (!ctx || !in || !out || M < 1) return fail(ctx, HANK_ERR_BAD_ARG, "hank_vjp_het: bad argument (M=%d)", M);
    const int rc = het_count_ok(ctx, "hank_vjp_het", n_het, true);
    if (rc) return rc;
    if (!ctx->primal_done) return fail(ctx, HANK_ERR_NOT_READY, "hank_primal must be called before hank_vjp_het");
    return HANK_OK;
}

// ... 89 lines not shown
    hipStream_t s = ctx->stream;
    Scratch sc;
    double *Vin, *xt, *sK, *kc, *A, *B, *u, *v, *pol, *Vout;
    int *ib;
    HIPC(ctx, sc.alloc(&Vin, G)); HIPC(ctx, sc.alloc(&xt, 3)); HIPC(ctx, sc.alloc(&sK, G)); HIPC(ctx, sc.alloc(&kc, G));
    HIPC(ctx, sc.alloc(&A, G)); HIPC(ctx, sc.alloc(&B, G)); HIPC(ctx, sc.alloc(&u, G)); HIPC(ctx, sc.alloc(&v, G));
    HIPC(ctx, sc.alloc(&pol, G)); HIPC(ctx, sc.alloc(&Vout, G)); HIPC(ctx, sc.alloc(&ib, G));
    if (!(1.0 + xhh_t[0] > 0.0)) return fail(ctx, HANK_ERR_DOMAIN, "1 + r must be positive");
    HIPC(ctx, hipMemcpyAsync(Vin, value_next, sizeof(double) * G, hipMemcpyHostToDevice, s));
    HIPC(ctx, hipMemcpyAsync(xt, xhh_t, sizeof(double) * c.n_hh, hipMemcpyHostToDevice, s));
    zero_err(ctx, s);
    const dim3 blk(RBP * c.n_e), grd(ctx->nbp);
    hipLaunchKernelGGL(k_egm_X, grd, blk, primal_lds(c), s, c, Vin, xt, sK, kc, ctx->d_err, 0, (const int *)nullptr);
    hipLaunchKernelGGL(k_egm_Y, grd, blk, 0, s, c, sK, xhh_t[0], xhh_t[1], c.n_hh > 2 ? xhh_t[2] : 0.0, pol, ib, A, B, u, v, Vout, ctx->d_err, 0, (const int *)nullptr);
    HIPC(ctx, hipGetLastError());
    const int rc = device_verdict(ctx, THIS_CALL);
    if (rc) return rc;
    HIPC(ctx, hipMemcpyAsync(value_out, Vout, sizeof(double) * G, hipMemcpyDeviceToHost, s));
    HIPC(ctx, hipMemcpyAsync(policy_out, pol, sizeof(double) * G, hipMemcpyDeviceToHost, s));
    if (N > 0) {
        double *dVin, *dr, *dw, *dtr = nullptr, *ds, *dpol, *dV;
        HIPC(ctx, sc.alloc(&dVin, G * N)); HIPC(ctx, sc.alloc(&dr, N)); HIPC(ctx, sc.alloc(&dw, N));
        HIPC(ctx, sc.alloc(&ds, G * N)); HIPC(ctx, sc.alloc(&dpol, G * N)); HIPC(ctx, sc.alloc(&dV, G * N));
        std::vector<double> hr(N), hw(N), ht(N);
        for (int n = 0; n < N; n++) { hr[n] = dxhh_t[c.n_hh * n]; hw[n] = dxhh_t[c.n_hh * n + 1]; ht[n] = c.n_hh > 2 ? dxhh_t[c.n_hh * n + 2] : 0.0; }
        if (c.n_hh > 2) {
            HIPC(ctx, sc.alloc(&dtr, N));
            HIPC(ctx, hipMemcpyAsync(dtr, ht.data(), sizeof(double) * N, hipMemcpyHostToDevice, s));
        }
        HIPC(ctx, hipMemcpyAsync(dVin, dvalue_next, sizeof(double) * G * N, hipMemcpyHostToDevice, s));
        HIPC(ctx, hipMemcpyAsync(dr, hr.data(), sizeof(double) * N, hipMemcpyHostToDevice, s));
        HIPC(ctx, hipMemcpyAsync(dw, hw.data(), sizeof(double) * N, hipMemcpyHostToDevice, s));
        const unsigned nb = (unsigned)((G * N + 255) / 256);
        hipLaunchKernelGGL(k_tan_X, dim3(nb), dim3(256), 0, s, c, kc, sK, xhh_t[0], dr, dw, dtr, N, dVin, ds);
        hipLaunchKernelGGL(k_tan_Y, dim3(nb), dim3(256), 0, s, c, ib, A, B, u, v, dr, dw, dtr, N, ds, dpol, dV);
        HIPC(ctx, hipGetLastError());
        HIPC(ctx, hipMemcpyAsync(dvalue_out, dV, sizeof(double) * G * N, hipMemcpyDeviceToHost, s));
        HIPC(ctx, hipMemcpyAsync(dpolicy_out, dpol, sizeof(double) * G * N, hipMemcpyDeviceToHost, s));
    }
    HIPC(ctx, hipStreamSynchronize(s));
    ctx->errmsg[0] = 0;
    return HANK_OK;
}

static int hx_outputs(hank_ctx *ctx, int NX, const TanBatch *b, double **T_out) {
    const Consts &c = ctx->c;
    const int N = b ? b->N : 0;
    const size_t P = c.P, G = c.G;
    const int nbr = (c.n_a + HX_ROWS - 1) / HX_ROWS;
    int rc = ensure_hx_record(ctx);
    if (rc) return rc;
    *T_out = nullptr;
    if (N == 0) return HANK_OK;
    const size_t sz[5] = {P * G * N, G * N, G * N, (size_t)N * P * nbr * NX, (size_t)N * P * NX};
    size_t need = 0, off = 0;
    for (size_t k : sz) carve(need, sizeof(double) * k);
    if (need > ctx->hx_bytes) {
        if (ctx->hx_slab) HIPC(ctx, hipStreamSynchronize(ctx->stream));
        ctx->hx_bytes = 0;
        HIPC(ctx, ctx->hx_slab.alloc(need));
        ctx->hx_bytes = need;
    }
    double *buf[5];
    for (int k = 0; k < 5; k++) buf[k] = reinterpret_cast<double *>(ctx->hx_slab + carve(off, sizeof(double) * sz[k]));
    double *dpc = buf[0], *mid = buf[1], *dD = buf[2], *parts = buf[3], *T = buf[4];
    rc = export_dpol_dev(ctx, *b, dpc);
    if (rc) return rc;
    const dim3 gmid((unsigned)((G + HX_ROWS - 1) / HX_ROWS), (unsigned)N), gmix((unsigned)nbr, (unsigned)N);
    for (size_t t = 0; t < P; t++) {
        hipLaunchKernelGGL(k_hx_mid, gmid, dim3(HX_ROWS), 0, ctx->stream, c, ctx->R, (int)t, dpc, dD, mid);
        hipLaunchKernelGGL(k_hx_mix, gmix, dim3(HX_ROWS), 0, ctx->stream, c, ctx->R, (int)t, NX, dpc, mid, ctx->hx.f.get(), ctx->hx.fc.get(), dD, parts);
    }
    const size_t cnt = (size_t)N * P * NX;
    hipLaunchKernelGGL(k_hx_reduce, dim3((unsigned)((cnt + 255) / 256)), dim3(256), 0, ctx->stream, parts, nbr, NX, cnt, T);
    HIPC(ctx, hipGetLastError());
    *T_out = T;
    return HANK_OK;
}

static int assemble_het_outputs(hank_ctx *ctx, int n_het, int Nk, const double *d_dx, const double *dagg_cm, const double *hxT, const double *bnd_zm, double *d_a, double *d_da) {
    const size_t P = ctx->c.P;
    const int nh = ctx->c.n_hh;
    hipLaunchKernelGGL(k_het_outputs, dim3((unsigned)((P * ((size_t)Nk + 1) + 255) / 256)), dim3(256), 0, ctx->stream, (int)P, nh, n_het, hx_count(ctx), Nk, ctx->d_xhh,
                       d_dx, ctx->d_agg, dagg_cm, ctx->d_zd, ctx->hx.S.get(), hxT, d_a, d_da);
    if (d_da && n_het >= 2 && bnd_zm)
        hipLaunchKernelGGL(k_bnd_cons, dim3((unsigned)((P * Nk + 255) / 256)), dim3(256), 0, ctx->stream, (int)P, nh, n_het, Nk, ctx->d_xhh, bnd_zm, d_da);
    HIPC(ctx, hipGetLastError());
    return HANK_OK;
}

static int het_outputs(hank_ctx *ctx, int32_t n_het, const double *dxhh, int32_t N, double *agg_out, double *dagg_out, bool dev) {
    if (!ctx) return HANK_ERR_BAD_ARG;
    ENTER(ctx);
    int rc = het_count_ok(ctx, "hank_get_het_outputs", n_het, true, N >= 0 && (agg_out || dagg_out));
    if (rc) return rc;
    if (!ctx->primal_done) return fail(ctx, HANK_ERR_NOT_READY, "no primal sweep has been run");
    const size_t P = ctx->c.P, nh = ctx->c.n_hh;
    const bool tan = dagg_out && N > 0;
    if (tan && !dxhh) return fail(ctx, HANK_ERR_BAD_ARG, "the tangent outputs need the dxhh of the last tangent sweep");
    const TanBatch *b = nullptr;
    if (tan) {
        rc = batch_current(ctx, N, &b);
        if (rc) return rc;
        if (b->boundary && n_het > 2)
            return fail(ctx, HANK_ERR_NOT_READY, "hank_get_het_outputs: the current tangent batch carries boundary seeds (hank_jvp_boundary), under which only outputs 0 and 1 "
                        "have tangents (Value and UCE assume dD_0 = 0): n_het = %d is served again after hank_jvp", n_het);
// ... 586 lines not shown
    if (!ctx || !out_ms) return HANK_ERR_BAD_ARG;
    ENTER(ctx);
    HIPC(ctx, hipStreamSynchronize(ctx->stream));
    for (int k = 0; k < 2; k++) HIPC(ctx, ctx->spans.read((Span)(SSB_VALUE + k), &out_ms[k], nullptr));
    return HANK_OK;
}
}

template <typename Step>
static int ss_loop(hank_ctx *ctx, SsCtl *d_ctl, int max_iter, Step step, SsCtl *out, Span span) {
    hipStream_t s = ctx->stream;
    SsCtl h{};
    HIPC(ctx, ctx->spans.begin(span, s));
    HIPC(ctx, hipMemsetAsync(d_ctl, 0, sizeof(SsCtl), s));
    int done = 0;
    const int chunk = 64;
    while (!h.stop && done < max_iter) {
        const int n = std::min(chunk, max_iter - done);
        for (int k = 0; k < n; k++) step(done + k);
        done += n;
        HIPC(ctx, hipGetLastError());
        HIPC(ctx, hipMemcpyAsync(&h, d_ctl, sizeof(SsCtl), hipMemcpyDeviceToHost, s));
        HIPC(ctx, hipStreamSynchronize(s));
    }
    HIPC(ctx, ctx->spans.end(span, s, 2 * done));
    *out = h;
    return HANK_OK;
}

static int ss_ready(hank_ctx *ctx, const char *name, int n_het, bool rest_ok) {
    int rc = het_count_ok(ctx, name, n_het, true, rest_ok);
    if (rc) return rc;
    rc = stationary_record(ctx, name);
    if (rc) return rc;
    if (ctx->c.P < 2) return fail(ctx, HANK_ERR_BAD_ARG, "%s needs a record of at least two periods (T >= 3)", name);
    return HANK_OK;
}

static int ss_jvp(hank_ctx *ctx, int n_het, const double *dxhh, int N, double tol, int max_iter, double *dvalue_out, double *dpolicy_out, double *dD_out,
                  double *dagg_out, int32_t *iters_out, double *resid_out, bool dev) {
    if (!ctx) return HANK_ERR_BAD_ARG;
    ENTER(ctx);
    int rc = ss_ready(ctx, "hank_ss_jvp", n_het, dxhh && dagg_out && iters_out && resid_out && N >= 1 && max_iter >= 1 && tol >= 0.0);
    if (rc) return rc;
    const Consts &c = ctx->c;
    const size_t G = c.G, GV = (size_t)(c.n_a + KV) * c.n_e, NN = (size_t)N;
    const int NX = n_het > 2 ? n_het - 2 : 0, V = (N % 2 == 0) ? 2 : 1;
    hipStream_t s = ctx->stream;
    const TanGeom g = tan_geom(c.n_a, N, V);
    TanGeom gf = g;
    gf.ss = g.NC >= 16 ? 1 : 0;
    const int RGB = 2, RGF = gf.ss ? 2 : 1;
    const unsigned nbt = (g.nbx + RGB - 1) / RGB, nbf = (gf.nbx + RGF - 1) / RGF + KV, ny = (g.N + g.NC - 1) / g.NC;
    { const int src = ensure_seg(ctx); if (src) return src; }
    { const int src = ensure_lwg(ctx); if (src) return src; }
    HIPC(ctx, join_side(ctx));
    if (NX > 0) { rc = ensure_hx_record(ctx); if (rc) return rc; }
    Scratch sc;
    double *dx, *dxr, *dxw, *dxt, *ds[2], *dV, *dpol, *dD[2], *aggpart, *hxparts, *partsB, *partsF, *sig, *out, *expV = nullptr, *expP = nullptr, *expD = nullptr;
    SsCtl *ctl;
    HIPC(ctx, sc.alloc(&dx, (size_t)c.n_hh * NN)); HIPC(ctx, sc.alloc(&dxr, 2 * NN)); HIPC(ctx, sc.alloc(&dxw, 2 * NN)); HIPC(ctx, sc.alloc(&dxt, 2 * NN));
    HIPC(ctx, sc.alloc(&ds[0], G * NN)); HIPC(ctx, sc.alloc(&ds[1], G * NN)); HIPC(ctx, sc.alloc(&dV, G * NN)); HIPC(ctx, sc.alloc(&dpol, 2 * G * NN));
    HIPC(ctx, sc.alloc(&dD[0], GV * NN)); HIPC(ctx, sc.alloc(&dD[1], GV * NN)); HIPC(ctx, sc.alloc(&aggpart, 2 * (size_t)nbf * NN));
    HIPC(ctx, sc.alloc(&hxparts, (size_t)nbf * (NX ? NX : 1) * NN)); HIPC(ctx, sc.alloc(&partsB, 2 * (size_t)nbt * NN));
    HIPC(ctx, sc.alloc(&partsF, 3 * (size_t)nbf * NN)); HIPC(ctx, sc.alloc(&sig, NN)); HIPC(ctx, sc.alloc(&out, (size_t)n_het * NN));
    HIPC(ctx, sc.alloc(&ctl, 2));
    if (!dev && dvalue_out) HIPC(ctx, sc.alloc(&expV, G * NN));
    if (!dev && dpolicy_out) HIPC(ctx, sc.alloc(&expP, G * NN));
    if (!dev && dD_out) HIPC(ctx, sc.alloc(&expD, G * NN));
    HIPC(ctx, hipMemcpyAsync(dx, dxhh, sizeof(double) * c.n_hh * NN, dev ? hipMemcpyDeviceToDevice : hipMemcpyHostToDevice, s));
    HIPC(ctx, hipMemsetAsync(ds[0], 0, sizeof(double) * G * NN, s));
    HIPC(ctx, hipMemsetAsync(dV, 0, sizeof(double) * G * NN, s));
    HIPC(ctx, hipMemsetAsync(dD[0], 0, sizeof(double) * GV * NN, s));
    hankss_launch_in(s, dx, c.n_hh, N, dxr, dxw, dxt);
    SsCtl hv{}, hd{};
    rc = ss_loop(ctx, &ctl[0], max_iter, [&](int k) {
        hankss_launch_back(s, V, c, ctx->R, ctx->d_xhh.get(), dxr, dxw, dxt, g, nbt, ny, ds[k & 1], ds[(k + 1) & 1], dpol, dV, partsB, &ctl[0]);
        hankss_launch_check(s, partsB, (int)nbt, 2, N, tol, &ctl[0], nullptr);
    }, &hv, SS_VALUE);
    if (rc) return rc;
    const double *dap = dpol + G * NN;
    rc = ss_loop(ctx, &ctl[1], max_iter, [&](int k) {
        hankss_launch_fwd(s, V, NX, c, ctx->R, gf, nbf, ny, dD[k & 1], dD[(k + 1) & 1], dap, aggpart, ctx->hx.f.get(), ctx->hx.fc.get(), hxparts, partsF, &ctl[1]);
        hankss_launch_check_dist(s, c, ctx->R.Dseq, partsF, (int)nbf, N, tol, dD[(k + 1) & 1], dD[k & 1], sig, &ctl[1]);
    }, &hd, SS_DIST);
    if (rc) return rc;
    const double *dDfin = dD[hd.iters & 1];
    hankss_launch_jvp_out(s, c.P, c.n_hh, n_het, N, (int)nbf, ctx->d_xhh.get(), dx, ctx->d_agg.get(), ctx->d_zd.get(), ctx->hx.S.get(), aggpart, hxparts, out);
    const dim3 tblk(BND_T, 8), tgrd((unsigned)((c.n_a + BND_T - 1) / BND_T), (unsigned)((N + BND_T - 1) / BND_T), (unsigned)c.n_e);
    const hipMemcpyKind back = dev ? hipMemcpyDeviceToDevice : hipMemcpyDeviceToHost;
    HIPC(ctx, hipMemcpyAsync(dagg_out, out, sizeof(double) * n_het * NN, back, s));
    if (dvalue_out) {
        hipLaunchKernelGGL(k_bnd_out, tgrd, tblk, 0, s, dV, c.n_a, c.n_e, N, dev ? dvalue_out : expV);
        if (!dev) HIPC(ctx, hipMemcpyAsync(dvalue_out, expV, sizeof(double) * G * NN, hipMemcpyDeviceToHost, s));
    }
    if (dpolicy_out) {
        hipLaunchKernelGGL(k_bnd_out, tgrd, tblk, 0, s, dap, c.n_a, c.n_e, N, dev ? dpolicy_out : expP);
        if (!dev) HIPC(ctx, hipMemcpyAsync(dpolicy_out, expP, sizeof(double) * G * NN, hipMemcpyDeviceToHost, s));
    }
    if (dD_out) {
        hankss_launch_dist_out(s, dDfin, c.n_a, c.n_e, N, dev ? dD_out : expD);
        if (!dev) HIPC(ctx, hipMemcpyAsync(dD_out, expD, sizeof(double) * G * NN, hipMemcpyDeviceToHost, s));
    }
    HIPC(ctx, hipGetLastError());
    HIPC(ctx, hipStreamSynchronize(s));
    iters_out[0] = hv.iters; iters_out[1] = hd.iters;
    resid_out[0] = hv.resid; resid_out[1] = hd.resid;
    ctx->errmsg[0] = 0;
    return HANK_OK;
}

static int ss_vjp_loops(hank_ctx *ctx, int V, const AdjGeom &g, int NX, double tol, int max_iter, double *e[2], double *lam, double *pbar, double *nu[2], const double *vbar,
                        const double *yb, double *partS, double *partM, double *parts, double *cen, SsCtl *ctl, SsCtl *hn, SsCtl *hl) {
    const Consts &c = ctx->c;
    hipStream_t s = ctx->stream;
    const int M = g.MV * V;
    const size_t ldsA = adj_lds_dist(c, g, V), ldsB = adj_lds_egm(c, g, V), PG = (size_t)c.P * c.G;
    const char *rce = getenv("HANK_SS_RECENTRE");
    const bool recentre = !(rce && atoi(rce) == 0);
    int rc = ss_loop(ctx, &ctl[1], max_iter, [&](int k) {
        hankss_launch_lam(s, V, false, ldsA, c, ctx->R, g, e[k & 1], e[(k + 1) & 1], lam, parts, &ctl[1], cen, nullptr, 0, nullptr, PG, nullptr);
        hankss_launch_check(s, parts, g.nb, 3, M, tol, &ctl[1], recentre ? cen : nullptr);
    }, hl, SS_DIST);
    if (rc) return rc;
    hankss_launch_lam(s, V, true, ldsA, c, ctx->R, g, lam, nullptr, nullptr, nullptr, nullptr, nullptr, yb, NX, ctx->hx.fc.get(), PG, pbar);
    return ss_loop(ctx, &ctl[0], max_iter, [&](int k) {
        hankss_launch_nu(s, V, ldsB, c, ctx->R, g, ctx->d_adj_sb.get(), nu[k & 1], nu[(k + 1) & 1], pbar, vbar, partS, partM, parts, &ctl[0]);
        hankss_launch_check(s, parts, g.nb, 2, M, tol, &ctl[0], nullptr);
    }, hn, SS_VALUE);
}

static int ss_vjp(hank_ctx *ctx, int n_het, const double *agg_bar, const double *value_bar, const double *D_bar, int M, double tol, int max_iter, double *xhh_bar,
                  int32_t *iters_out, double *resid_out, bool dev) {
    if (!ctx) return HANK_ERR_BAD_ARG;
    ENTER(ctx);
    if (!agg_bar && !value_bar && !D_bar) return fail(ctx, HANK_ERR_BAD_ARG, "hank_ss_vjp: agg_bar, value_bar and D_bar are all NULL: nothing to pull back");
    int rc = ss_ready(ctx, "hank_ss_vjp", n_het, xhh_bar && iters_out && resid_out && M >= 1 && max_iter >= 1 && tol >= 0.0);
    if (rc) return rc;
    const Consts &c = ctx->c;
    const size_t G = c.G, MM = (size_t)M;
    const int NX = n_het > 2 ? n_het - 2 : 0, V = adj_lane_width(M);
    hipStream_t s = ctx->stream;
    const AdjGeom g = adj_geom(c.n_a, M);
    if (adj_lds_dist(c, g, V) > ctx->lds_max || adj_lds_egm(c, g, V) > ctx->lds_max)
        return fail(ctx, HANK_ERR_BAD_ARG, "hank_ss_vjp: n_e=%d needs more LDS per workgroup than the device has", c.n_e);
    if (!ctx->d_adj_sb) HIPC(ctx, ctx->d_adj_sb.alloc((size_t)c.P * c.n_e * ((size_t)c.n_a + 1)));
    HIPC(ctx, join_side(ctx));
    rc = ensure_adj_seg(ctx);
    if (rc) return rc;
    if (NX > 0) { rc = ensure_hx_record(ctx); if (rc) return rc; }
    Scratch sc;
    double *ybar = nullptr, *stage = nullptr, *yb, *e[2], *lam, *pbar, *nu[2], *vbar = nullptr, *partS, *partM, *parts, *xbar, *cen;
    SsCtl *ctl;
    const hipMemcpyKind in = dev ? hipMemcpyDeviceToDevice : hipMemcpyHostToDevice;
    HIPC(ctx, sc.alloc(&yb, 4 * MM)); HIPC(ctx, sc.alloc(&e[0], G * MM)); HIPC(ctx, sc.alloc(&e[1], G * MM)); HIPC(ctx, sc.alloc(&lam, G * MM));
    HIPC(ctx, sc.alloc(&pbar, G * MM)); HIPC(ctx, sc.alloc(&nu[0], G * MM)); HIPC(ctx, sc.alloc(&nu[1], G * MM));
    HIPC(ctx, sc.alloc(&partS, 3 * (size_t)g.nb * MM)); HIPC(ctx, sc.alloc(&partM, 3 * (size_t)g.nb * MM)); HIPC(ctx, sc.alloc(&parts, 3 * (size_t)g.nb * MM)); HIPC(ctx, sc.alloc(&cen, MM));
    HIPC(ctx, sc.alloc(&xbar, (size_t)c.n_hh * MM)); HIPC(ctx, sc.alloc(&ctl, 2));
    if (agg_bar) {
        HIPC(ctx, sc.alloc(&ybar, (size_t)n_het * MM));
        HIPC(ctx, hipMemcpyAsync(ybar, agg_bar, sizeof(double) * n_het * MM, in, s));
    }
    hankss_launch_y_in(s, ybar, n_het, M, yb);
    const dim3 tblk(BND_T, 8), tgrd((unsigned)((c.n_a + BND_T - 1) / BND_T), (unsigned)((M + BND_T - 1) / BND_T), (unsigned)c.n_e);
    if (value_bar || D_bar) HIPC(ctx, sc.alloc(&stage, G * MM));
    if (value_bar) {
        HIPC(ctx, sc.alloc(&vbar, G * MM));
        HIPC(ctx, hipMemcpyAsync(stage, value_bar, sizeof(double) * G * MM, in, s));
        hipLaunchKernelGGL(k_bnd_in, tgrd, tblk, 0, s, (const double *)stage, c.n_a, c.n_e, c.n_a, M, vbar);
    }
    if (D_bar) HIPC(ctx, hipMemcpyAsync(stage, D_bar, sizeof(double) * G * MM, in, s));
    hankss_launch_cot_in(s, c, ctx->R, ctx->d_xhh.get(), NX, yb, D_bar ? stage : nullptr, ctx->hx.f.get(), (size_t)c.P * G, M, e[0], lam);
    HIPC(ctx, hipMemsetAsync(nu[0], 0, sizeof(double) * G * MM, s));
    HIPC(ctx, hipMemsetAsync(cen, 0, sizeof(double) * MM, s));
    SsCtl hn{}, hl{};
    rc = ss_vjp_loops(ctx, V, g, NX, tol, max_iter, e, lam, pbar, nu, vbar, yb, partS, partM, parts, cen, ctl, &hn, &hl);
    if (rc) return rc;
    hankss_launch_xbar(s, c.P, c.n_hh, M, g.nb, NX, ctx->d_xhh.get(), partS, partM, yb, ctx->d_agg.get(), ctx->d_zd.get(), ctx->hx.S.get(), xbar);
    HIPC(ctx, hipGetLastError());
    HIPC(ctx, hipMemcpyAsync(xhh_bar, xbar, sizeof(double) * c.n_hh * MM, dev ? hipMemcpyDeviceToDevice : hipMemcpyDeviceToHost, s));
    HIPC(ctx, hipStreamSynchronize(s));
    iters_out[0] = hn.iters; iters_out[1] = hl.iters;
    resid_out[0] = hn.resid; resid_out[1] = hl.resid;
    ctx->errmsg[0] = 0;
    return HANK_OK;
}

extern "C" {
int hank_ss_jvp(hank_ctx *ctx, int32_t n_het, const double *dxhh, int32_t N, double tol, int32_t max_iter, double *dvalue_out, double *dpolicy_out, double *dD_out,
                double *dagg_out, int32_t *iters_out, double *resid_out) {
    return ss_jvp(ctx, n_het, dxhh, N, tol, max_iter, dvalue_out, dpolicy_out, dD_out, dagg_out, iters_out, resid_out, false);
}
int hank_ss_jvp_dev(hank_ctx *ctx, int32_t n_het, const double *d_dxhh, int32_t N, double tol, int32_t max_iter, double *d_dvalue_out, double *d_dpolicy_out,
                    double *d_dD_out, double *d_dagg_out, int32_t *iters_out, double *resid_out) {
    return ss_jvp(ctx, n_het, d_dxhh, N, tol, max_iter, d_dvalue_out, d_dpolicy_out, d_dD_out, d_dagg_out, iters_out, resid_out, true);
}
int hank_ss_vjp(hank_ctx *ctx, int32_t n_het, const double *agg_bar, const double *value_bar, const double *D_bar, int32_t M, double tol, int32_t max_iter,
                double *xhh_bar, int32_t *iters_out, double *resid_out) {
    return ss_vjp(ctx, n_het, agg_bar, value_bar, D_bar, M, tol, max_iter, xhh_bar, iters_out, resid_out, false);
}
// ... 13 lines not shown
```

julia-newtonraphsonhank_amd/csrc/hank_kernels.h:

```cpp
#pragma once
#include <hip/hip_runtime.h>
#include <stdint.h>
#include "hank_device.h"

namespace hank {

constexpr int RBP = 32;


template <int CRRA = 0>
__device__ inline bool pow_domain_error(double v, double y) {
    if constexpr (CRRA == 1) return (v < 0.0) && (y == -0.5);
    else return (v < 0.0) && (y != floor(y));
}

__device__ __forceinline__ double fast_rcp(double x) {
    double r = __builtin_amdgcn_rcp(x);
    r = __builtin_fma(__builtin_fma(-x, r, 1.0), r, r);
    r = __builtin_fma(__builtin_fma(-x, r, 1.0), r, r);
    return r;
}
__device__ __forceinline__ double fast_rsqrt(double x) {
    double y = __builtin_amdgcn_rsq(x);
    y = __builtin_fma(y * 0.5, __builtin_fma(-(x * y), y, 1.0), y);
// ... 233 lines not shown
__global__ void k_egm_Y(Consts c, const double *s, double r, double w, double tr, double *pol, int *ib,
                        double *A, double *B, double *u, double *v, double *Vout, int *err, int t, const int *stop) {
    if (stop && *stop) return;
    const int row = threadIdx.x % RBP, e = threadIdx.x / RBP;
    const int a = blockIdx.x * RBP + row;
    if (a >= c.n_a) return;
    const YOut o = egm_Y(c, s + e * c.n_a, a, e, r, w, tr, err, t, -1);
    const int off = e * c.n_a + a;
    pol[off] = o.g; ib[off] = o.ib; A[off] = o.A; B[off] = o.B; u[off] = o.u; v[off] = o.v;
    Vout[off] = o.V;
}

__device__ inline void egm_step_body(const Consts &c, const Record &R, const double *xhh, int t, int *err, int bid, double *sh) {
    double *Vsh = sh, *Pish = sh + c.n_e * RBP;
    const int nthr = RBP * c.n_e;
    const int row = threadIdx.x % RBP, e = threadIdx.x / RBP;
    const int a = bid * RBP + row;
    for (int k = threadIdx.x; k < c.n_e * c.n_e; k += nthr) Pish[k] = c.Pi[k];
    const size_t base = (size_t)t * c.G;
    if (a < c.n_a) {
        const double r = xhh[c.n_hh * t], w = xhh[c.n_hh * t + 1], tr = hh_tr(c, xhh, t);
        const int guess = (t + 1 < c.P) ? R.ib[base + c.G + (size_t)e * c.n_a + a] : -1;
        const YOut o = egm_Y(c, R.s + base + (size_t)e * c.n_a, a, e, r, w, tr, err, t, guess);
        const size_t off = base + (size_t)e * c.n_a + a;
        R.pol[off] = o.g; R.ib[off] = o.ib; R.A[off] = o.A;
        R.B[off] = o.B; R.u[off] = o.u; R.v[off] = o.v;
        Vsh[e * RBP + row] = o.V;
    }
    lds_barrier();
    if (t > 0 && a < c.n_a) {
        const double r1 = xhh[c.n_hh * (t - 1)], w1 = xhh[c.n_hh * (t - 1) + 1], tr1 = hh_tr(c, xhh, t - 1);
        const size_t off1 = base - c.G + (size_t)e * c.n_a + a;
        egm_X(c, Vsh, Pish, row, a, e, r1, w1, tr1, &R.s[off1], &R.kc[off1], err, t - 1);
    }
}
__global__ void k_egm_step(Consts c, Record R, const double *xhh, int t, int *err) {
    extern __shared__ double sh[];
    egm_step_body(c, R, xhh, t, err, blockIdx.x, sh);
}

__global__ void k_lottery(Consts c, Record R, int ncols, int *err, int write_seg, int use_ib) {
    extern __shared__ int shlo[];
    __shared__ int sh_clo;
    const int col = blockIdx.x;
    if (col >= ncols) return;
    lottery_body(c, R, col, err, write_seg, use_ib, shlo, &sh_clo);
}
#if HANK_XFWD_LQ
__global__ void k_lottery_lq(Consts c, Record R, int ncols, int *err, int write_seg, int use_ib, int4 *lq) {
    extern __shared__ int shlo[];
    __shared__ int sh_clo;
    const int col = blockIdx.x;
    if (col >= ncols) return;
    lottery_body(c, R, col, err, write_seg, use_ib, shlo, &sh_clo, lq);
}
__global__ void k_iga_build(Consts c, double *iga) {
    const int l = blockIdx.x * blockDim.x + threadIdx.x;
    if (l < c.n_a) iga[l] = l + 1 < c.n_a ? 1.0 / (c.a[l + 1] - c.a[l]) : 0.0;
}
#endif
__global__ void k_seg_build(Consts c, Record R, int ncols) {
    const int col = blockIdx.x, n = c.n_a;
    if (col >= ncols) return;
    const int *st = R.start + (size_t)col * (n + 1);
    const size_t base = (size_t)col * n;
    for (int r = threadIdx.x; r < n; r += blockDim.x)
        R.seg[base + r] = make_int4(r > 0 ? st[r - 1] : st[r], st[r], st[r + 1], 0);
}

__device__ inline void dist_step_body(const Consts &c, const Record &R, int t, double *aggpart, int bid, int nblocks, double *sh,
                                      const double *Din = nullptr, double *Dout = nullptr) {
    double *Dsh = sh, *Pish = sh + c.n_e * RBP, *red = Pish + c.n_e * c.n_e;
    const int nthr = RBP * c.n_e;
    const int row = threadIdx.x % RBP, e = threadIdx.x / RBP;
    const int r = bid * RBP + row;
    const int n = c.n_a;
    for (int k = threadIdx.x; k < c.n_e * c.n_e; k += nthr) Pish[k] = c.Pi[k];
    const double *Dprev = Din ? Din : R.Dseq + (size_t)t * c.G;
    const size_t base = (size_t)t * c.G;
    const double *lw = R.lw + base + (size_t)e * n, *Dp = Dprev + (size_t)e * n;
    double acc = 0.0;
    if (r < n) {
        if (!Din) R.lwg[base + (size_t)e * n + r] = make_double2(lw[r], R.ig[base + (size_t)e * n + r] * Dp[r]);
        const int *st = R.start + ((size_t)t * c.n_e + e) * (n + 1);
        const int st1 = st[r], st2 = st[r + 1], st0 = r > 0 ? st[r - 1] : st1;
        for (int j = st0; j < st1; j++) acc += lw[j] * Dp[j];
        for (int j = st1; j < st2; j++) acc += (1.0 - lw[j]) * Dp[j];
    }
    if (bid == 0) {
        const int clo = R.clo[(size_t)t * c.n_e + e];
        double part = 0.0;
        for (int j = row; j < clo; j += RBP) part += Dp[j];
#pragma unroll
        for (int off = 16; off > 0; off >>= 1) part += __shfl_xor(part, off, 64);
        if (row == 0) acc += part;
    }
    if (r < n) Dsh[e * RBP + row] = acc;
    lds_barrier();
    double part = 0.0, part2 = 0.0;
    if (r < n) {
        const int e2 = e;
        double Dn = 0.0;
        Dn = mix_sum(Dn, Dsh + row, RBP, Pish + c.n_e * e2, 1, 0, c.n_e);
        (Dout ? Dout[(size_t)e2 * n + r] : R.Dseq[(size_t)(t + 1) * c.G + (size_t)e2 * n + r]) = Dn;
        part = R.pol[base + (size_t)e2 * n + r] * Dn;
        part2 = c.a[r] * Dn;
    }
// ... 262 lines not shown
```

julia-newtonraphsonhank_amd/csrc/hank_xsweep.h:

```cpp
#pragma once
#include "hank_kernels.h"
#include "hank_xaddr.h"
#include "hank_xlds.h"
#include <type_traits>

namespace hank {

constexpr int XG = 8;
constexpr int XRW = 63;
enum { XERR_TIMEOUT = 1, XERR_PLACEMENT = 2 };
__device__ unsigned long long g_xwait_ticks = 2000000ull;
struct XDeadline {
    unsigned long long t0;
    __device__ __forceinline__ XDeadline() : t0(__builtin_amdgcn_s_memrealtime()) {}
    __device__ __forceinline__ bool expired(unsigned spins) const { return (spins & 63u) == 63u && __builtin_amdgcn_s_memrealtime() - t0 > g_xwait_ticks; }
    __device__ __forceinline__ unsigned waited_us() const { return (unsigned)((__builtin_amdgcn_s_memrealtime() - t0) / 100ull); }
};

struct XSync {
    unsigned ticket[XG][32];
    unsigned total[32];
    unsigned flag[XG][64][32];
    unsigned status[32];
    unsigned pad[32];
// ... 150 lines not shown
    if ((int)threadIdx.x < count) { base[threadIdx.x].status[0] = code; base[threadIdx.x].status[1] = 0u; }
}

__device__ __forceinline__ XMember xmember_join(XSync *sy, int *ctl, int groups, int n_a) {
    if (threadIdx.x == 0) {
        int xcc;
        asm volatile("s_getreg_b32 %0, hwreg(HW_REG_XCC_ID)" : "=s"(xcc));
        xcc &= 7;
        if (xldu(&sy->status[0]) != 0u) {
            ctl[0] = xcc; ctl[1] = 0; ctl[2] = 0; ctl[3] = 0;
        } else {
            const unsigned c = __hip_atomic_fetch_add(&sy->ticket[xcc][0], 1u, __ATOMIC_RELAXED, __HIP_MEMORY_SCOPE_AGENT);
            asm volatile("s_waitcnt vmcnt(0)" ::: "memory");
            __hip_atomic_fetch_add(&sy->total[0], 1u, __ATOMIC_RELAXED, __HIP_MEMORY_SCOPE_AGENT);
            int ok = 1;
            const XDeadline dl;
            for (unsigned spins = 0;; spins++) {
                if (xldu(&sy->total[0]) >= gridDim.x) break;
                if (dl.expired(spins) || ((spins & 255u) == 255u && xldu(&sy->status[0]) != 0u)) { xfail(sy, XERR_TIMEOUT, xcc, dl.waited_us()); ok = 0; break; }
                __builtin_amdgcn_s_sleep(2);
            }
            ctl[0] = xcc; ctl[1] = (int)c; ctl[2] = (int)xldu(&sy->ticket[xcc][0]); ctl[3] = ok;
        }
    }
    __syncthreads();
    XMember m;
    m.x = __builtin_amdgcn_readfirstlane(ctl[0]); m.c = __builtin_amdgcn_readfirstlane(ctl[1]);
    const int S = __builtin_amdgcn_readfirstlane(ctl[2]), ok = __builtin_amdgcn_readfirstlane(ctl[3]);
    m.Sact = (n_a + XRW - 1) / XRW;
    m.on = false;
    if (!ok || m.x >= groups) return m;
    if (S < m.Sact) { if (threadIdx.x == 0) xfail(sy, XERR_PLACEMENT, m.x); return m; }
    m.on = m.c < m.Sact;
    return m;
}
__device__ __forceinline__ XRoles xroles(int ne) {
    XRoles r;
    r.lane = threadIdx.x & 63; r.wv = __builtin_amdgcn_readfirstlane((int)(threadIdx.x >> 6));
    r.syncw = r.wv >= ne;
    r.sync_duty = blockDim.x > 64 * ne ? r.syncw : r.wv == 0;
    r.e = r.syncw ? 0 : r.wv;
    return r;
}

__device__ __forceinline__ void xlds_barrier() { asm volatile("s_waitcnt lgkmcnt(0)\n\ts_barrier" ::: "memory"); }

__device__ __forceinline__ void xbar_arrive(bool drain) {
    if (drain) asm volatile("s_waitcnt vmcnt(0)" ::: "memory");
    xlds_barrier();
}
__device__ __forceinline__ void xpublish(XSync *sy, int x, int c, unsigned episode) {
    if ((threadIdx.x & 63) == 0) *reinterpret_cast<volatile unsigned *>(&sy->flag[x][c][0]) = episode;
}
__device__ __forceinline__ void xpoll(XSync *sy, int x, int lo, int hi, unsigned need) {
    const int lane = threadIdx.x & 63;
    const XDeadline dl;
    for (unsigned spins = 0;; spins++) {
        const unsigned f = (lane >= lo && lane <= hi) ? xldu(&sy->flag[x][lane][0]) : need;
        if (__all((int)(f - need) >= 0)) break;
        if (dl.expired(spins) || ((spins & 255u) == 255u && xldu(&sy->status[0]) != 0u)) {
            if (lane == 0) xfail(sy, XERR_TIMEOUT, x, dl.waited_us());
            break;
        }
        __builtin_amdgcn_s_sleep(1);
    }
}
__device__ __forceinline__ void xbar_wait(XSync *sy, int x, int c, int members, unsigned episode, bool sync_wave) {
    if (sync_wave) { xpublish(sy, x, c, episode); xpoll(sy, x, 0, members - 1, episode); }
    xlds_barrier();
}

template <bool BUF>
struct XKnotsT {
    const double *p;
    __amdgpu_buffer_rsrc_t rs;
    int so;
    int a, n, i0, i1, i2, i3;
    double sa, sam1, s0, sN, w0, w1, w2, w3;
    double ze;
    __device__ __forceinline__ double ld(int i) const {
        if constexpr (BUF) return buf_ld64<16>(rs, i * 8, so);
        else return xld(p + i);
    }
    __device__ __forceinline__ void preload(const double *col, int a_, int n_, int guess, double ze_) { p = col; batch(a_, n_, guess, ze_); }
    __device__ __forceinline__ void preload(__amdgpu_buffer_rsrc_t rs_, int so_, int a_, int n_, int guess, double ze_) { rs = rs_; so = so_; batch(a_, n_, guess, ze_); }
    __device__ __forceinline__ void batch(int a_, int n_, int guess, double ze_) {
        a = a_; n = n_; ze = ze_;
        sa = ld(a);
        sam1 = ld(a > 0 ? a - 1 : 0);
        s0 = ld(0);
        sN = ld(n - 1);
        i0 = i1 = i2 = i3 = -1;
        w0 = w1 = w2 = w3 = 0.0;
        if (guess >= 0) {
            const int q = guess < n - 1 ? guess : n - 2;
            i0 = q > 0 ? q - 1 : 0; i1 = q; i2 = q + 1; i3 = q + 2 < n ? q + 2 : n - 1;
            w0 = ld(i0); w1 = ld(i1); w2 = ld(i2); w3 = ld(i3);
        }
    }
    __device__ __forceinline__ YFront front(double x, int guess) const {
        YFront f;
        f.bad = a > 0 ? !(sa > sam1) : !(sa == sa);
        const bool below = x < s0, above = !below & (x > sN);
        const int p = i1;
        const bool c0 = (w1 <= x) & (x < w2);
        const bool cp = !c0 & (p + 2 < n) & (w2 <= x) & (x < w3);
        const bool cm = !c0 & !cp & (p > 0) & (w0 <= x) & (x < w1);
        f.slow = !below & !above & ((guess < 0) | !(c0 | cp | cm));
        f.where = below ? Y_BELOW : (above ? Y_ABOVE : Y_INSIDE);
        f.i = c0 ? p : (cp ? p + 1 : p - 1);
        f.si = c0 ? w1 : (cp ? w2 : w0);
        f.sj = c0 ? w2 : (cp ? w3 : w1);
        return f;
    }
    __device__ __forceinline__ double column_z() const { return ze; }
    __device__ __forceinline__ double operator[](int i) const {
        if (i == a) return sa;
        if (i == a - 1) return sam1;
        if (i == i1) return w1;
        if (i == i2) return w2;
        if (i == i0) return w0;
// ... 180 lines not shown
    extern __shared__ __attribute__((aligned(16))) double xl[];
    const Consts &c = A.c;
    const int ne = c.n_e, na = c.n_a, P = c.P, G = c.G;
    const XLdsPrimalBack L = xlds_primal_back(ne, na, P);
    double *Vsh = xlds_at<double>(xl, L.Vsh), *Pish = xlds_at<double>(xl, L.Pish), *ash = xlds_at<double>(xl, L.ash), *xsh = xlds_at<double>(xl, L.xsh);
    int *ctl = xlds_at<int>(xl, L.ctl);
    const XMember mb = xmember_join(A.sy, ctl, 1, na);
    if (!mb.on) return;
    const int x = mb.x, cW = mb.c, Sact = mb.Sact;
    const XRoles rl = xroles(ne);
    const int lane = rl.lane, e = rl.e; const bool syncw = rl.syncw, sync_duty = rl.sync_duty;
    const int a = cW * XRW + lane;
    const bool own = !syncw && lane < XRW && a < na;
    const size_t pt = (size_t)e * na + (own ? a : 0);
    for (int k = threadIdx.x; k < ne * ne; k += blockDim.x) Pish[k] = c.Pi[k];
    for (int k = threadIdx.x; k < na; k += blockDim.x) ash[k] = c.a[k];
    xstage_prices(xsh, c, A.xhh, A.rho, P);
    Consts cl = c;
    cl.a = ash;
    const double ze = c.z[e], xa = c.a[own ? a : 0];
    const size_t hs = (size_t)XG * G;
    double *const sS = A.st_s;
    if (!syncw) Vsh[e * 64 + lane] = own ? A.ss_value[pt] : 0.0;
    __syncthreads();
    int guess = -1;
    unsigned episode = 0;
    for (int i = 0; i <= P; i++) {
        if (i > 0) {
            const int t = P - i, cur = (i - 1) & 1;
            double V = 0.0;
            if (own) {
                XKnots kn;
                kn.preload(sS + (size_t)cur * hs + (size_t)e * na, a, na, guess, ze);
                const YOut o = egm_Y(cl, kn, a, e, xsh[4 * t], xsh[4 * t + 1], xsh[4 * t + 2], A.err, t, guess);
                guess = o.ib;
                V = o.V;
                const size_t ro = (size_t)t * G + pt;
                A.R.pol[ro] = o.g; A.R.ib[ro] = o.ib; A.R.A[ro] = o.A; A.R.B[ro] = o.B; A.R.u[ro] = o.u; A.R.v[ro] = o.v;
            }
            if (!syncw) Vsh[e * 64 + lane] = V;
            xlds_barrier();
        }
        if (i < P) {
            const int tx = P - 1 - i;
            if (own) {
                double E;
                xtile_mix<1, 1>(Vsh + lane, Pish + e, ne, ne, &E);
                const XPoint p = egm_X_point(c, E, xsh + 4 * tx, ze, xa, A.err, tx, e, a);
                sS[(size_t)(i & 1) * hs + pt] = p.s1;
                A.R.s[(size_t)tx * G + pt] = p.s1; A.R.kc[(size_t)tx * G + pt] = p.kc;
            }
            episode++;
            xbar_arrive(!syncw);
            xbar_wait(A.sy, x, cW, Sact, episode, sync_duty);
        }
    }
}
static inline size_t x_lds_primal_back(const Consts &c) { return xlds_primal_back(c.n_e, c.n_a, c.P).bytes; }

struct XVfiArgs {
    Consts c;
    const double *V0;
    double r, w, tr;
    double tol;
    int max_iter;
    XSync *sy;
    double *st_s;
    int *err;
    double *Vout, *pol;
    int *iters;
    double *supnorm;
};

template <int MAXT>
__global__ void __launch_bounds__(MAXT) k_xvfi(XVfiArgs A) {
    extern __shared__ __attribute__((aligned(16))) double xl[];
    const Consts &c = A.c;
    const int ne = c.n_e, na = c.n_a, G = c.G;
    const XLdsVfi L = xlds_vfi(ne, na);
    double *Vsh = xlds_at<double>(xl, L.Vsh), *Pish = xlds_at<double>(xl, L.Pish), *ash = xlds_at<double>(xl, L.ash), *redsh = xlds_at<double>(xl, L.redsh);
    int *ctl = xlds_at<int>(xl, L.ctl);
    const XMember mb = xmember_join(A.sy, ctl, 1, na);
    if (!mb.on) return;
    const int x = mb.x, cW = mb.c, Sact = mb.Sact;
    const XRoles rl = xroles(ne);
    const int lane = rl.lane, wv = rl.wv, e = rl.e; const bool syncw = rl.syncw, sync_duty = rl.sync_duty;
    const int a = cW * XRW + lane;
    const bool own = !syncw && lane < XRW && a < na;
    const size_t pt = (size_t)e * na + (own ? a : 0);
    for (int k = threadIdx.x; k < ne * ne; k += blockDim.x) Pish[k] = c.Pi[k];
    for (int k = threadIdx.x; k < na; k += blockDim.x) ash[k] = c.a[k];
    Consts cl = c;
    cl.a = ash;
    const double ze = c.z[e], xa = c.a[own ? a : 0];
    const double x4[4] = {A.r, A.w, A.tr, 1.0 / (1.0 + A.r)};
    const size_t hs = (size_t)XG * G;
    double *const sS = A.st_s;
    double Vprev = own ? A.V0[pt] : 0.0, V = Vprev, pol = 0.0;
    if (!syncw) Vsh[e * 64 + lane] = Vprev;
    __syncthreads();
    int guess = -1, steps = 0, conv = 0;
    double gmax = 0.0;
    unsigned episode = 0;
    for (int i = 0; i <= A.max_iter; i++) {
        double dmax = 0.0;
        if (i > 0) {
            const int cur = (i - 1) & 1;
// ... 31 lines not shown
}
static inline size_t x_lds_vfi(const Consts &c) { return xlds_vfi(c.n_e, c.n_a).bytes; }


struct XStatArgs {
    Consts c;
    Record R;
    const double *D0;
    double tol;
    int max_iter, check_every;
    XSync *sy;
    double *st_D;
    double *Dout;
    int *iters;
};

template <int MAXT>
__global__ void __launch_bounds__(MAXT) k_xstat(XStatArgs A) {
    extern __shared__ __attribute__((aligned(16))) double xl[];
    const Consts &c = A.c;
    const Record &R = A.R;
    const int ne = c.n_e, na = c.n_a, G = c.G;
    const int GV = G + 64 * ne;
    const XLdsStat L = xlds_stat(ne);
    double *tile = xlds_at<double>(xl, L.tile), *redsh = xlds_at<double>(xl, L.redsh);
    int *ctl = xlds_at<int>(xl, L.ctl);
    const XMember mb = xmember_join(A.sy, ctl, 1, na);
    if (!mb.on) return;
    const int x = mb.x, cW = mb.c, Sact = mb.Sact;
    const XRoles rl = xroles(ne);
    const int lane = rl.lane, wv = rl.wv, e = rl.e; const bool syncw = rl.syncw, sync_duty = rl.sync_duty;
    const int r0 = cW * XRW, r = r0 + lane;
    const bool own = !syncw && lane < XRW && r < na;
    const bool virt = !syncw && lane == 63;
    const size_t pt = (size_t)e * na + (own ? r : 0);
    const size_t slot = own ? pt : (size_t)G + (size_t)e * 64 + cW;
    double pr[16];
#pragma unroll
    for (int k = 0; k < 16; k++) pr[k] = k < ne ? c.Pi[ne * e + k] : 0.0;
    const size_t hs = (size_t)XG * GV;
    double *const sP = A.st_D;
    double Dcur = own ? A.D0[pt] : 0.0;
    if (own || virt) sP[slot] = Dcur;
    double Dchk = Dcur;
    int sg0 = 0, sg1 = 0, sg2 = 0;
    if (own) { const int4 q = R.seg[pt]; sg0 = q.x; sg1 = q.y; sg2 = q.z; }
    const int clo = syncw ? 0 : min(max(R.clo[e], 0), na);
    bool anyclo = false;
    for (int k = 0; k < ne; k++) anyclo = anyclo || R.clo[k] > 0;
    const int s0 = max(sg0, 0), s2 = min(sg2, na);
    const bool need_vD = anyclo && clo == 0 && __any(own && (sg0 <= 0 && s2 > 0));
    unsigned episode = 1;
    xbar_arrive(!syncw);
    xbar_wait(A.sy, x, cW, Sact, episode, sync_duty);
    int cur = 0, it = 0, conv = 0;
    bool vnz = false;
    for (it = 1; it <= A.max_iter; it++) {
        const size_t hb = (size_t)cur * hs;
        double accD = 0.0;
        if (!syncw) {
            const double *Dp = sP + hb + (size_t)e * na;
            double cD = 0.0;
            if (own && r < clo) cD = xld(Dp + r);
            if (virt && clo > 0 && vnz) cD = xld(sP + hb + slot);
            double vD = 0.0;
            if (vnz && need_vD) {
                if (lane < Sact) vD = xld(sP + hb + (size_t)G + (size_t)e * 64 + lane);
                vD = xwave_sum(vD);
            }
            if (own) {
                for (int j0 = s0; j0 < s2; j0 += 4) {
                    double wj[4], Dj[4];
                    bool on[4];
#pragma unroll
                    for (int u = 0; u < 4; u++) {
                        const int j = j0 + u;
                        on[u] = j < s2;
                        wj[u] = 0.0; Dj[u] = 0.0;
                        if (on[u]) { wj[u] = R.lw[(size_t)e * na + j]; Dj[u] = xld(Dp + j); }
                    }
#pragma unroll
                    for (int u = 0; u < 4; u++) {
                        const int j = j0 + u;
                        if (!on[u]) continue;
                        if (j == 0) Dj[u] += vD;
                        accD += (j < sg1 ? wj[u] : 1.0 - wj[u]) * Dj[u];
                    }
                }
            }
            if (clo > r0) cD = xwave_reduce63(cD);
            if (virt) accD = cD;
            tile[e * 64 + lane] = accD;
        }
        xlds_barrier();
        vnz = anyclo;
        const int nxt = cur ^ 1;
        const bool chk = (it % A.check_every) == 0 || it == A.max_iter;
        double dmax = 0.0;
        if (!syncw) {
            double Dn;
            xtile_mix_reg<1, 1>(tile + lane, pr, ne, &Dn);
            if (own || virt) sP[(size_t)nxt * hs + slot] = Dn;
            Dcur = Dn;
            if (chk) {
                if (own) dmax = fabs(Dn - Dchk);
                else if (virt) dmax = fabs(Dn - Dchk) * (double)Sact;
                Dchk = Dn;
// ... 44 lines not shown
    const Record &R = A.R;
    const int ne = c.n_e, na = c.n_a, P = c.P, G = c.G;
    const XLdsTanBack L = xlds_tan_back(ne, P, D);
    double *tile = xlds_at<double>(xl, L.tile), *rhosh = xlds_at<double>(xl, L.rhosh), *pxsh = xlds_at<double>(xl, L.pxsh), *dxsh = xlds_at<double>(xl, L.dxsh);
    int *srcsh = xlds_at<int>(xl, L.srcsh), *ctl = xlds_at<int>(xl, L.ctl);
    const XMember mb = xmember_join(A.sy, ctl, A.groups, na);
    if (!mb.on) return;
    const int x = mb.x, cW = mb.c, Sact = mb.Sact;
    for (int k = threadIdx.x; k < P; k += blockDim.x) { rhosh[k] = A.rho[k]; pxsh[3 * k] = 1.0 + A.xhh[c.n_hh * k]; pxsh[3 * k + 1] = A.xhh[c.n_hh * k + 1]; pxsh[3 * k + 2] = hh_tr(c, A.xhh, k); }
    for (int k = threadIdx.x; k < P; k += blockDim.x) srcsh[k] = A.src ? A.src[(size_t)k * Sact + cW] : ((Sact - 1) << 8);
    xstage_dx<D>(dxsh, c, A.dxr, A.dxw, A.dxt, A.Ntot, A.n0, A.N, x, P);
    const XRoles rl = xroles(ne);
    const int lane = rl.lane, e = rl.e; const bool syncw = rl.syncw, sync_duty = rl.sync_duty;
    const int r0 = cW * XRW, a = r0 + lane;
    const bool own = !syncw && lane < XRW && a < na;
    const size_t pt = (size_t)e * na + (own ? a : 0);
    const double ze = c.z[e], xa = c.a[own ? a : 0];
    const size_t hs = (size_t)XG * G;
    XRows<D> rows;
    rows.init(A.st_ds, 2 * hs);
    const size_t gx = (size_t)x * G;
    double *const myt = tile + ((size_t)e * 64 + lane) * SL;
    {
        double z[D];
#pragma unroll
        for (int k = 0; k < D; k++) z[k] = 0.0;
        if (!syncw) xtile_store_n<SL, D>(myt, z);
    }
    __syncthreads();
    double pr[16];
#pragma unroll
    for (int k = 0; k < 16; k++) pr[k] = k < ne ? c.Pi[e + ne * k] : 0.0;
    int ibY = 0;
    double cA = 0.0, cB = 0.0, cu = 0.0, cv = 0.0, ck = 0.0, cs = 0.0;
    if (own) { cs = R.s[(size_t)(P - 1) * G + pt]; if (!c.diet) ck = R.kc[(size_t)(P - 1) * G + pt]; }
    int n_ib = 0;
    double n_A = 0.0, n_B = 0.0, n_u = 0.0, n_v = 0.0, n_k = 0.0, n_s = 0.0;
    auto load_next = [&](int ty) {
        if (own && ty >= 0) {
            const size_t ro = (size_t)ty * G + pt;
            n_ib = R.ib[ro]; n_A = R.A[ro]; n_B = R.B[ro]; n_u = R.u[ro];
            if (!c.diet) n_v = R.v[ro];
            if (ty > 0) { n_s = R.s[ro - G]; if (!c.diet) n_k = R.kc[ro - G]; }
        }
    };
    constexpr bool DEEP = D <= 2;
    if constexpr (DEEP) load_next(P - 1);
    const int son = (x == 0 && cW < 32) ? cW : -1;
    (void)son;
    for (int i = 0; i <= P; i++) {
        XSTAMP(0, son, i, 0);
        if (i > 0) {
            const int t = P - i, cur = (i - 1) & 1;
            if (sync_duty) xpoll(A.sy, x, srcsh[t] & 255, srcsh[t] >> 8, (unsigned)i);
            xlds_barrier();
            XSTAMP(0, son, i, 1);
            double dV[D];
#pragma unroll
            for (int k = 0; k < D; k++) dV[k] = 0.0;
            if (own) {
                double d0[D], d1[D], dg[D];
#pragma unroll
                for (int k = 0; k < D; k++) d0[k] = d1[k] = 0.0;
                if (cA != 0.0 || cB != 0.0) {
                    const size_t rb = (size_t)cur * hs + gx + (size_t)e * na;
                    rows.load(rb + ibY, d0);
                    rows.load(rb + ibY + 1, d1);
                }
                const double cvt = c.diet ? diet_v(c, cu, pxsh[3 * t]) : cv;
#pragma unroll
                for (int k = 0; k < D; k++) {
                    const double dr = dxsh[(t * 3 + 0) * D + k], dw = dxsh[(t * 3 + 1) * D + k], dtr = dxsh[(t * 3 + 2) * D + k];
                    dg[k] = cA * d0[k] + cB * d1[k];
                    dV[k] = cu * dr + cvt * ((xa * dr + (ze * dw + dtr)) - dg[k]);
                }
                xstore_row<D>(A.dpol + (((size_t)t * A.groups + x) * G + pt) * D, dg);
            }
            if (!syncw) xtile_store_n<SL, D>(myt, dV);
            XSTAMP(0, son, i, 2);
            XSTAMPV(0, son, i);
            if (sync_duty) xpoll(A.sy, x, 0, Sact - 1, (unsigned)i);
            xlds_barrier();
            XSTAMP(0, son, i, 3);
        }
        if (i < P) {
            const int tx = P - 1 - i;
            if (own) {
                const double rho = rhosh[tx];
                const double ckt = c.diet ? diet_kc(c, cs, rho, pxsh[3 * tx], pxsh[3 * tx + 1] * ze + pxsh[3 * tx + 2], xa) : ck;
                double mx[D], ds[D];
                xtile_mix_reg<SL, D>(tile + (size_t)lane * SL, pr, ne, mx);
#pragma unroll
                for (int k = 0; k < D; k++) {
                    const double dr1 = dxsh[(tx * 3 + 0) * D + k], dw1 = dxsh[(tx * 3 + 1) * D + k], dt1 = dxsh[(tx * 3 + 2) * D + k];
                    ds[k] = ckt * mx[k] - rho * ((ze * dw1 + dt1) + cs * dr1);
                }
                rows.store((size_t)(i & 1) * hs + gx + pt, ds);
            }
            XSTAMP(0, son, i, 4);
            xbar_arrive(!syncw);
            XSTAMP(0, son, i, 5);
            if (sync_duty && !(A.stall && x == 0 && cW == 0 && i > 2)) xpublish(A.sy, x, cW, (unsigned)(i + 1));
            if constexpr (DEEP) {
                ibY = n_ib; cA = n_A; cB = n_B; cu = n_u; cv = n_v;
                if (tx > 0) { cs = n_s; ck = n_k; }
                load_next(tx - 1);
            } else if (own) {
                const size_t ro = (size_t)tx * G + pt;
                ibY = R.ib[ro]; cA = R.A[ro]; cB = R.B[ro]; cu = R.u[ro];
                if (!c.diet) cv = R.v[ro];
                if (tx > 0) { cs = R.s[ro - G]; if (!c.diet) ck = R.kc[ro - G]; }
            }
        }
    }
}
static inline size_t x_lds_tan_back(const Consts &c, int D) { return xlds_tan_back(c.n_e, c.P, D).bytes; }

struct XDualBackArgs {
    XBackArgs p;
    const double *dxr, *dxw, *dxt;
    int Ntot, n0, N;
    double *st_ds;
    double *dpol;
    int groups;
    XRecOff ro;
    unsigned dpol_bytes;
};

template <int D, int MAXT, int NE = 0, int CRRA = 0>
__global__ void __launch_bounds__(MAXT) k_xdual_back(XDualBackArgs B) {
    constexpr int NSL = D + 1, SL = XSlots<NSL>::SL, IV = D;
    extern __shared__ __attribute__((aligned(16))) double xl[];
    const XBackArgs &A = B.p;
    const Consts &c = A.c;
// ... 83 lines not shown
                        for (int k = 0; k < D; k++) d1[k] = w0[k];
                        rows.load_vs(o.ib, icb, d0);
                    } else {
                        rows.load_vs(o.ib, icb, d0); rows.load_vs(o.ib + 1, icb, d1);
                    }
                }
#pragma unroll
                for (int k = 0; k < D; k++) {
                    const double dr = dxsh[(t * 3 + 0) * D + k], dw = dxsh[(t * 3 + 1) * D + k], dtr = dxsh[(t * 3 + 2) * D + k];
                    dg[k] = o.A * d0[k] + o.B * d1[k];
                    tv[k] = o.u * dr + o.v * ((xa * dr + (ze * dw + dtr)) - dg[k]);
                }
                xstore_row_buf<D>(rdp, ipt * (8 * D), (int)((unsigned)((t * B.groups + x) * G) * (unsigned)(8 * D)), dg);
                const int tg = t * G, rcm = xopaque(rcm0);
                if (rcm & 1) buf_st64<0>(o.g, rrec, ipt * 8, (int)(B.ro.pol + (unsigned)tg * 8u));
                if (rcm & 2) buf_st32<0>(o.ib, rrec, ipt * 4, (int)(B.ro.ib + (unsigned)tg * 4u));
                if (rcm & 4) buf_st64<0>(o.A, rrec, ipt * 8, (int)(B.ro.A + (unsigned)tg * 8u));
                if (rcm & 8) buf_st64<0>(o.B, rrec, ipt * 8, (int)(B.ro.B + (unsigned)tg * 8u));
                if (rcm & 16) buf_st64<0>(o.u, rrec, ipt * 8, (int)(B.ro.u + (unsigned)tg * 8u));
                if (rcm & 32) buf_st64<0>(o.v, rrec, ipt * 8, (int)(B.ro.v + (unsigned)tg * 8u));
            }
            if (!syncw) xtile_store_n<SL, NSL>(myt, tv);
            XSTAMP(0, son, i, 2);
            XSTAMPV(0, son, i);
            xlds_barrier();
            XSTAMP(0, son, i, 3);
        }
        if (i < P) {
            const int tx = P - 1 - i;
            if (own) {
                double mx[NSL];
                constexpr bool STEPS = CRRA == 0 && NE * ((NSL + 1) / 2) > 24;
                if constexpr (NE > 0 && STEPS) xtile_mix_reg<SL, NSL, false, true, NK>(tile + (size_t)lane * SL, pr, xopaque(NE), mx);
                else if constexpr (NE > 0) xtile_mix_reg<SL, NSL, false, false, NK>(tile + (size_t)lane * SL, pr, NE, mx);
                else xtile_mix_reg<SL, NSL, false, true>(tile + (size_t)lane * SL, pr, xopaque(ne), mx);
                const XPoint p = egm_X_point<CRRA>(c, mx[IV], xsh + 4 * tx, ze, xa, A.err, tx, e, a);
                const double s1 = p.s1, kc = p.kc, rho = xsh[4 * tx + 3];
                double ds[D];
#pragma unroll
                for (int k = 0; k < D; k++) {
                    const double dr1 = dxsh[(tx * 3 + 0) * D + k], dw1 = dxsh[(tx * 3 + 1) * D + k], dt1 = dxsh[(tx * 3 + 2) * D + k];
                    ds[k] = kc * mx[k] - rho * ((ze * dw1 + dt1) + s1 * dr1);
                }
                const int ihb = (i & 1) * ihs + igx, rcm = xopaque(rcm0);
                buf_st64<0>(s1, rkn, ipt * 8, ihb * 8);
                rows.store_vs(ipt, ihb, ds);
                if (rcm & 64) buf_st64<0>(s1, rrec, ipt * 8, (int)(B.ro.s + (unsigned)(tx * G) * 8u));
                if (rcm & 128) buf_st64<0>(kc, rrec, ipt * 8, (int)(B.ro.kc + (unsigned)(tx * G) * 8u));
            }
            episode++;
            XSTAMP(0, son, i, 4);
            xbar_arrive(!syncw);
            XSTAMP(0, son, i, 5);
            xbar_wait(A.sy, x, cW, Sact, episode, sync_duty);
        }
    }
    XSTAMP1(0, son, 11);
}
static inline size_t x_lds_dual_back(const Consts &c, int D) { return xlds_dual_back(c.n_e, c.n_a, c.P, D).bytes; }

constexpr int XUCAP = 64;
struct XSweepFwdArgs {
    Consts c;
    Record R;
    XSync *sy;
    double *st;
    const double *D0;
    const double *dpol;
    int groups;
    double *Dvirt;
    double *aggpart;
    double *daggpart;
    const int *src;
    const int *overflow;
    const int2 *units;
    int all_members;
    XRecOff ro;
    unsigned dpol_bytes;
    unsigned iga;
};

#if HANK_XFWD_LQ
template <int D, bool VAL, int MAXT, bool LQ = false>
#else
template <int D, bool VAL, int MAXT>
#endif
__global__ void __launch_bounds__(MAXT) k_xfwd(XSweepFwdArgs A) {
#pragma clang fp contract(fast)
#if !HANK_XFWD_LQ
    constexpr bool LQ = false;
#endif
    constexpr int NSL = D + (VAL ? 1 : 0);
    constexpr int SP = XSlots<NSL>::SP, SL = XSlots<NSL>::SL;
    constexpr int IV = D;
    constexpr int DD = D > 0 ? D : 1;
    constexpr bool PIREG = NSL < 4;
    constexpr bool XB = VAL && D > 0;
    constexpr bool EARLYB = XB && HANK_XFWD_EARLY_BATCH != 0;
    static_assert(!LQ || XB, "the packed record is read through the record's descriptor");
    extern __shared__ __attribute__((aligned(16))) double xl[];
    const Consts &c = A.c;
    const Record &R = A.R;
    const int ne = c.n_e, na = c.n_a, P = c.P, G = c.G;
    const XLdsFwd L = xlds_fwd(ne, P, D, VAL);
    double *tile = xlds_at<double>(xl, L.tile), *Pish = xlds_at<double>(xl, L.Pish), *aggsh = xlds_at<double>(xl, L.aggsh);
    constexpr int NAP = 2 * NSL;
    int *closh = xlds_at<int>(xl, L.closh), *srcsh = xlds_at<int>(xl, L.srcsh), *ctl = xlds_at<int>(xl, L.ctl);
// ... 152 lines not shown
        request_units(t + 2);
    };
    xbar_arrive(!syncw);
    if (sync_duty) xpublish(A.sy, x, cW, 1u);
    ud[0] = ud[1] = make_int2(0, 0);
    if (!syncw) { request_units(0); take_units(); load_rec(I0, 0, ud[0], 0); load_rec(I1, 0, ud[1], 0); prefetch(0); request_units(1); }
    int cur = 0;
    bool vnz = false;
    const int son = (x == 0 && cW < 32) ? cW : -1;
    (void)son;
    auto reduce_agg = [&](int tp) {
        const double *ap = aggsh + (size_t)lane * NAP;
        double sk[NAP];
#pragma unroll
        for (int k = 0; k < NAP; k++) sk[k] = 0.0;
        for (int k2 = 0; k2 < ne; k2++) {
            double v[NAP];
            if (NAP == 1) v[0] = ap[(size_t)k2 * 64 * NAP];
            else {
#pragma unroll
                for (int q = 0; q < NAP / 2; q++) { const double2 d = reinterpret_cast<const double2 *>(ap + (size_t)k2 * 64 * NAP)[q]; v[2 * q] = d.x; v[2 * q + 1] = d.y; }
            }
#pragma unroll
            for (int k = 0; k < NAP; k++) sk[k] += v[k];
        }
        const size_t pb = (size_t)tp * Sact + cW;
#pragma unroll
        for (int k = 0; k < D; k++) {
            const double pd = xwave_reduce63(sk[k]), pd2 = xwave_reduce63(sk[NSL + k]);
            if (lane == 63) { A.daggpart[pb * (size_t)(2 * XG * D) + x * D + k] = pd; A.daggpart[pb * (size_t)(2 * XG * D) + XG * D + x * D + k] = pd2; }
        }
        if constexpr (VAL) {
            if (recD) {
                const double pD = xwave_reduce63(sk[IV]), pD2 = xwave_reduce63(sk[NSL + IV]);
                if (lane == 63) { A.aggpart[2 * pb] = pD; A.aggpart[2 * pb + 1] = pD2; }
            }
        }
    };
    for (int t = 0; t < P; t++) {
        XSTAMP(1, son, t, 0);
        const size_t base = (size_t)t * G + (size_t)e * na;
        const size_t hb = (size_t)cur * hs;
        const int sw = srcsh[t];
        int clo = 0;
        if (!syncw) {
            clo = min(max(closh[t * ne + e], 0), na);
            double z[SL];
#pragma unroll
            for (int k = 0; k < SL; k++) z[k] = 0.0;
            xtile_store<SL>(myt, z);
            set_g(I0);
            set_g(I1);
        }
        if (sync_duty) xpoll(A.sy, x, sw & 255, (sw >> 8) & 255, (unsigned)(t + 1));
        xlds_barrier();
        XSTAMP(1, son, t, 1);
        if (sync_duty && t > 0) reduce_agg(t - 1);
        double pagg[DD];
#pragma unroll
        for (int k = 0; k < DD; k++) pagg[k] = 0.0;
        double v0 = 0.0;
        if (!syncw) {
            const bool need0 = recL && r0 == 0 && vnz && clo == 0;
            if constexpr (RECL) {
                if (need0 && lane < Sact) v0 = rows.load_one(hb + gx + ((size_t)e * Sact + lane) * 64 + 63, IV);
            }
            load_state(I0, hb, cur, ud[0], 0);
            load_state(I1, hb, cur, ud[1], 0);
            auto process_pc = [&](auto U, int2 d) {
                constexpr int u = decltype(U)::value;
                const int ta = d.y & 0xff, tb = (d.y >> 8) & 0xff;
                double *const colt = tile + (size_t)(d.x & 15) * 64 * SL;
                const double w = qw[u], w1 = 1.0 - w;
                double gD = qg[u], Dv = 0.0;
                if constexpr (VAL) { Dv = dd[u][IV]; gD = qg[u] * Dv; }
                else { if (qvl[u]) gD = 0.0; }
                const int tl = qlo[u] - r0, th = tl + 1;
                const bool doL = qon[u] && tl >= ta && tl < tb, doH = qon[u] && th >= ta && th < tb;
                const int thp = __builtin_amdgcn_update_dpp(-2, doH ? th : -2, 0x138, 0xf, 0xf, false);
                const bool take = doL && thp == tl;
                const bool given = __builtin_amdgcn_update_dpp(0, take ? 1 : 0, 0x130, 0xf, 0xf, false) != 0;
                double *const tpl = colt + (size_t)(doL ? tl : 0) * SL, *const tph = colt + (size_t)(doH ? th : 0) * SL;
#pragma unroll
                for (int k = 0; k < D; k++) {
                    const double hk = w * dd[u][k] + gD * qdp[u][k];
                    const double hp = xdpp<0x138, 0xf, 0xf>(hk);
                    const double lk = w1 * dd[u][k] - gD * qdp[u][k];
                    if (doL) lds_add(tpl + k, take ? lk + hp : lk);
                    if (doH && !given) lds_add(tph + k, hk);
                }
                if constexpr (VAL) {
                    if (doL) lds_add(tpl + IV, w1 * Dv);
                    if (doH) lds_add(tph + IV, w * Dv);
                }
                if constexpr (!VAL) {
                    if (doL && !qvl[u]) {
#pragma unroll
                        for (int k = 0; k < D; k++) pagg[k] += qdp[u][k] * qdn[u];
                    }
                }
            };
            auto process_1 = [&](auto U, int2 d) {
                constexpr int u = decltype(U)::value;
                if (!qon[u]) return;
                const int ta = d.y & 0xff, tb = (d.y >> 8) & 0xff;
                double *const colt = tile + (size_t)(d.x & 15) * 64 * SL;
                const double w = qw[u], w1 = 1.0 - w;
                double gD = qg[u], Dv = 0.0;
                if constexpr (VAL) { Dv = dd[u][IV]; gD = qg[u] * Dv; }
                else { if (qvl[u]) gD = 0.0; }
                const int tl = qlo[u] - r0, th = tl + 1;
                if (tl >= ta && tl < tb) {
                    double *tp = colt + (size_t)tl * SL;
#pragma unroll
                    for (int k = 0; k < D; k++) lds_add(tp + k, w1 * dd[u][k] - gD * qdp[u][k]);
                    if constexpr (VAL) lds_add(tp + IV, w1 * Dv);
                    if constexpr (!VAL) {
                        if (!qvl[u]) {
#pragma unroll
                            for (int k = 0; k < D; k++) pagg[k] += qdp[u][k] * qdn[u];
                        }
                    }
                }
                if (th >= ta && th < tb) {
                    double *tp = colt + (size_t)th * SL;
#pragma unroll
                    for (int k = 0; k < D; k++) lds_add(tp + k, w * dd[u][k] + gD * qdp[u][k]);
                    if constexpr (VAL) lds_add(tp + IV, w * Dv);
                }
            };
            constexpr bool PRECOMB = NSL >= 3;
            auto process = [&](auto U, int2 d) { if constexpr (PRECOMB) process_pc(U, d); else process_1(U, d); };
            process(I0, ud[0]);
            process(I1, ud[1]);
            const int nu = (sw >> 18) & 0xff;
            for (int u2 = wv; u2 < nu; u2 += ne) {
                const int2 d = u2 < 2 * ne ? ud[u2 >= ne ? 1 : 0] : unit_desc(t, u2);
                const int tot = ((d.x >> 16) & 0xfff) + ((d.y >> 16) & 0xff);
                for (int i0 = u2 < 2 * ne ? 64 : 0; i0 < tot; i0 += 64) {
                    load_rec(I0, t, d, i0);
                    load_state(I0, hb, cur, d, i0);
                    set_g(I0);
                    process(I0, d);
                }
            }
            if constexpr (RECL) { if (need0) v0 = xwave_sum(v0); }
            take_units();
            if constexpr (EARLYB) next_units_loads(t);
            XSTAMP(1, son, t, 2);
            double cT[NSL];
#pragma unroll
            for (int k = 0; k < NSL; k++) cT[k] = ((own && r < clo) || (virt && clo > 0 && vnz)) ? mxp[k] : 0.0;
            if (clo > r0) {
#pragma unroll
                for (int k = 0; k < NSL; k++) cT[k] = xwave_reduce63(cT[k]);
            }
            if (virt) xtile_store_n<SL, NSL>(myt, cT);
        }
        XSTAMP(1, son, t, 3);
        XSTAMPV(1, son, t);
        if (sync_duty) xpoll(A.sy, x, 0, Sact - 1, (unsigned)(t + 1));
        xlds_barrier();
        XSTAMP(1, son, t, 4);
        vnz = ((sw >> 16) & 1) != 0;
        const int nxt = cur ^ 1;
        if (!syncw) {
            if constexpr (!EARLYB) next_units_loads(t);
            double mx[NSL];
            if (PIREG) xtile_mix_reg<SL, NSL, true>(tile + (size_t)lane * SL, pr, ne, mx);
            else xtile_mix<SL, NSL, true>(tile + (size_t)lane * SL, Pish + ne * e, 1, ne, mx);
            if (live) {
                double sv[SP];
#pragma unroll
                for (int k = 0; k < SP; k++) sv[k] = k < NSL ? mx[k] : 0.0;
                if constexpr (XB) rows.store_vs(lane, nxt * ihs + igx + islot, sv);
                else rows.store((size_t)nxt * hs + slot, sv);
            }
            double at[NAP];
#pragma unroll
            for (int k = 0; k < NAP; k++) at[k] = 0.0;
            if constexpr (RECL) {
                if (recL && own) {
                    double Dfull = mxp[IV];
                    if (r == 0 && clo == 0) Dfull += v0;
                    R.lwg[base + r] = make_double2(lwr, igr * Dfull);
                }
            }
            if constexpr (VAL) {
                if (recD) {
                    if (own) {
                        if constexpr (XB) buf_st64<0>(mx[IV], rrec, ipt * 8, (int)(A.ro.Dseq + (unsigned)((t + 1) * G) * 8u));
                        else R.Dseq[(size_t)(t + 1) * G + pt] = mx[IV];
                    } else if (virt) A.Dvirt[((size_t)t * ne + e) * 64 + cW] = mx[IV];
                    at[IV] = live ? polr * mx[IV] : 0.0;
                    at[NSL + IV] = live ? xar * mx[IV] : 0.0;
                }
            }
#pragma unroll
            for (int k = 0; k < D; k++) {
                double term = live ? polr * mx[k] : 0.0;
                if constexpr (VAL) term = live ? (polr * mx[k] + dpr[k] * mx[IV]) : 0.0;
                else term = (term + pagg[k]) + ((own && r < clo) ? dpr[k] * Dr : 0.0);
                at[k] = term;
                at[NSL + k] = live ? xar * mx[k] : 0.0;
            }
            xtile_store<NAP>(aggsh + ((size_t)e * 64 + lane) * NAP, at);
#pragma unroll
            for (int k = 0; k < NSL; k++) mxp[k] = mx[k];
        }
        cur = nxt;
        XSTAMP(1, son, t, 5);
        if (!syncw) {
            asm volatile("; XFWD_BATCH_BEGIN" ::: "memory");
            prefetch(min(t + 1, P - 1));
// ... 245 lines not shown
```

Before: 9201 JVPs/s.

## Defer unpacked lottery record writes and add pipelined flag polling option

After: 9275 JVPs/s, median of 6. About the same (+0.8%).

```diff
diff --git a/julia-newtonraphsonhank_amd/csrc/hank_device.h b/julia-newtonraphsonhank_amd/csrc/hank_device.h
--- a/julia-newtonraphsonhank_amd/csrc/hank_device.h
+++ b/julia-newtonraphsonhank_amd/csrc/hank_device.h
@@ -8,6 +8,12 @@
 #endif
 #ifndef HANK_XFWD_EARLY_BATCH
 #define HANK_XFWD_EARLY_BATCH 0
+#endif
+#ifndef HANK_LOTTERY_LAZY
+#define HANK_LOTTERY_LAZY 1
+#endif
+#ifndef HANK_XPOLL_DEPTH
+#define HANK_XPOLL_DEPTH 1
 #endif
 
 namespace hank {
@@ -525,6 +531,7 @@
     }
 }
 
+template <bool LQ_ONLY = false>
 __device__ __forceinline__ void lottery_body(const Consts &c, const Record &R, int col, int *err, int write_seg, int use_ib, int *shlo, int *sh_clo, int4 *lq = nullptr) {
     const int t = col / c.n_e, e = col % c.n_e;
     const size_t base = (size_t)col * c.n_a;
@@ -557,7 +564,8 @@
             w = (p - c.a[l]) / gap;
             ig = 1.0 / gap;
         }
-        R.lo[base + j] = l; R.lw[base + j] = w; R.ig[base + j] = ig;
+        if constexpr (!LQ_ONLY) { R.lo[base + j] = l; R.lw[base + j] = w; R.ig[base + j] = ig; }
+        else (void)ig;
         if (lq) lq[base + j] = make_int4(__double2loint(w), __double2hiint(w), l, (hi == 0 || hi >= n) ? 1 : 0);
         shlo[j] = (hi == 0) ? -1 : l;
     }
diff --git a/julia-newtonraphsonhank_amd/csrc/hank_hip.hip b/julia-newtonraphsonhank_amd/csrc/hank_hip.hip
--- a/julia-newtonraphsonhank_amd/csrc/hank_hip.hip
+++ b/julia-newtonraphsonhank_amd/csrc/hank_hip.hip
@@ -232,6 +232,7 @@
     bool seg_valid = true;
     bool lwg_valid = true;
     long long lwg_builds = 0;
+    bool lot_valid = true;
     bool wprep_valid = false;
     std::list<WTan> wtans;
     std::list<CotWork> cws;
@@ -276,14 +277,14 @@
     *out = &ctx->batch;
     return HANK_OK;
 }
-static void record_rewritten(hank_ctx *ctx, bool seg_written, bool lwg_written) {
-    ctx->primal_done = true; ctx->seg_valid = seg_written; ctx->lwg_valid = lwg_written;
+static void record_rewritten(hank_ctx *ctx, bool seg_written, bool lwg_written, bool lot_written) {
+    ctx->primal_done = true; ctx->seg_valid = seg_written; ctx->lwg_valid = lwg_written; ctx->lot_valid = lot_written;
     ctx->wprep_valid = false; ctx->xw.src_valid = false; ctx->xw.rng_valid = false; ctx->adj_seg_valid = false; ctx->hx.valid = false;
     batch_none(ctx);
     cot_none(ctx);
 }
 static void record_gone(hank_ctx *ctx) {
-    record_rewritten(ctx, false, false);
+    record_rewritten(ctx, false, false, false);
     ctx->primal_done = false;
 }
 static hipError_t join_side(hank_ctx *ctx) {
@@ -840,10 +841,17 @@
     else if (sp.ne == 11) by_crra(std::integral_constant<int, 11>());
     else by_crra(std::integral_constant<int, 0>());
 }
+static bool x_fwd_reads_lq(const XWork &X, const Consts &c, int D) {
+#if HANK_XFWD_LQ
+    return D > 0 && x_lds_fwd_lq(c, D) <= (size_t)X.lds_max;
+#else
+    return false;
+#endif
+}
 static void x_launch_fwd(XSection &sec, XWork &X, const Consts &c, int D, bool val, const XSweepFwdArgs &a) {
     if (val && D > 0) { X.inst[2] = 0; X.inst[3] = 0; }
 #if HANK_XFWD_LQ
-    if (val && D > 0 && x_lds_fwd_lq(c, D) <= (size_t)X.lds_max) {
+    if (val && x_fwd_reads_lq(X, c, D)) {
         const size_t lds = x_lds_fwd_lq(c, D);
         x_by_maxt(X, [&](auto mt) {
             constexpr int MT = decltype(mt)::value;
@@ -888,8 +896,24 @@
     ctx->seg_valid = true;
     return HANK_OK;
 }
+#if HANK_XFWD_LQ
+constexpr bool X_LOTTERY_LAZY = HANK_LOTTERY_LAZY != 0;
+#else
+constexpr bool X_LOTTERY_LAZY = false;
+#endif
+static int ensure_lot(hank_ctx *ctx) {
+    if (ctx->lot_valid) return HANK_OK;
+#if HANK_XFWD_LQ
+    const size_t npt = (size_t)ctx->c.P * ctx->c.G;
+    hipLaunchKernelGGL(k_lottery_unpack, dim3((unsigned)((npt + 255) / 256)), dim3(256), 0, ctx->stream, ctx->R, ctx->rec_lq, ctx->rec_iga, ctx->c.n_a, npt);
+    HIPC(ctx, hipGetLastError());
+#endif
+    ctx->lot_valid = true;
+    return HANK_OK;
+}
 static int ensure_lwg(hank_ctx *ctx) {
     if (ctx->lwg_valid) return HANK_OK;
+    { const int rc = ensure_lot(ctx); if (rc) return rc; }
     const XWork &X = ctx->xw;
     hipLaunchKernelGGL(k_xlwg_build, dim3((unsigned)(ctx->c.P * ctx->c.n_e)), dim3(256), 0, ctx->stream, ctx->c, ctx->R, X.Dvirt, X.D0own, X.Sact);
     HIPC(ctx, hipGetLastError());
@@ -1012,6 +1036,7 @@
 static int x_tan_fwd(XSection &sec, XTan *w, int p, bool val) {
     hank_ctx *ctx = sec.ctx; XWork &X = ctx->xw;
     const XPass &ps = w->passes[p];
+    if (!(val && x_fwd_reads_lq(X, ctx->c, ps.D))) { const int rc = ensure_lot(ctx); if (rc) return rc; }
     if (!val) { const int rc = ensure_lwg(ctx); if (rc) return rc; }
     XSweepFwdArgs fa = x_fwd_args(ctx, val);
     fa.sy = X.sync + 2 + 2 * p + 1; fa.st = X.st_dD; fa.daggpart = w->daggpart; fa.groups = ps.groups; fa.dpol = w->dpol + ps.dpol_off;
@@ -1446,7 +1471,7 @@
     HIPC(ctx, hipEventRecord(ctx->ev_side, ctx->side_stream));
     ctx->side_pending = true;
     ctx->spans.invalidate({DUAL_BACK, DUAL_FWD});
-    record_rewritten(ctx, true, true);
+    record_rewritten(ctx, true, true, true);
     return HANK_OK;
 }
 
@@ -1460,7 +1485,7 @@
     x_rho(sec);
     rc = x_back(sec); if (rc) return rc;
     x_lottery(sec, true);
-    record_rewritten(ctx, true, true);
+    record_rewritten(ctx, true, true, true);
     x_ensure_rng(sec);
     rc = x_fwd_value(sec); if (rc) return rc;
     HIPC(ctx, hipGetLastError());
@@ -1512,7 +1537,7 @@
     x_rho(sec);
     rc = x_back(sec); if (rc) return rc;
     x_lottery(sec, true, true);
-    record_rewritten(ctx, true, false);
+    record_rewritten(ctx, true, false, !X_LOTTERY_LAZY);
     x_ensure_rng(sec);
     rc = x_tan_front(sec, w);
     if (!rc) rc = x_tan_back(sec, w);
@@ -1556,7 +1581,7 @@
     }
     int rc = x_back(sec, w); if (rc) return rc;
     x_lottery(sec, false, true);
-    record_rewritten(ctx, false, false);
+    record_rewritten(ctx, false, false, !X_LOTTERY_LAZY);
     x_ensure_rng(sec);
     HIPC(ctx, ctx->spans.begin(TAN_BACK, sec.stream()));
     HIPC(ctx, ctx->spans.end(TAN_BACK, sec.stream(), 1));
@@ -1648,6 +1673,7 @@
     HIPC(ctx, hipGraphLaunch(w.tan_back(bnd), ctx->stream));
     HIPC(ctx, ctx->spans.end(TAN_BACK, ctx->stream, ctx->c.P + (bnd ? 4 : 2)));
     HIPC(ctx, join_side(ctx));
+    { const int src = ensure_lot(ctx); if (src) return src; }
     { const int src = ensure_seg(ctx); if (src) return src; }
     { const int src = ensure_lwg(ctx); if (src) return src; }
     HIPC(ctx, ctx->spans.begin(TAN_FWD, ctx->stream));
@@ -1808,7 +1834,7 @@
     HIPC(ctx, hipGraphLaunch(w.g_ffwd, ctx->stream));
     HIPC(ctx, ctx->spans.end(DUAL_FWD, ctx->stream, ctx->c.P + 5));
     ctx->spans.invalidate({PRIMAL_BACK, PRIMAL_FWD, TAN_BACK, TAN_FWD});
-    record_rewritten(ctx, true, true);
+    record_rewritten(ctx, true, true, true);
     batch_ran(ctx, 0, &w, w.N, w.dagg_cm, w.dpol);
     return HANK_OK;
 }
@@ -1926,6 +1952,7 @@
     const Consts &c = ctx->c;
     const int P = c.P, G = c.G, N = c.n_hh, NP = P * N, S = 16, nh = n_het ? n_het : 1;
     hipStream_t s = ctx->stream;
+    { const int src = ensure_lot(ctx); if (src) return src; }
     { const int src = ensure_seg(ctx); if (src) return src; }
     { const int src = ensure_lwg(ctx); if (src) return src; }
     TanWork *wp = nullptr;
@@ -2082,6 +2109,7 @@
     if (!ctx->primal_done) return fail(ctx, HANK_ERR_NOT_READY, "no primal sweep has been run");
     if ((lq || iga) && !ctx->rec_lq) return fail(ctx, HANK_ERR_BAD_ARG, "hank_get_lottery_record: this build keeps no packed lottery record");
     HIPC(ctx, join_side(ctx));
+    if (lo || lw || ig) { const int rc = ensure_lot(ctx); if (rc) return rc; }
     const size_t n = (size_t)ctx->c.P * ctx->c.G;
     if (lo) HIPC(ctx, hipMemcpyAsync(lo, ctx->R.lo, sizeof(int) * n, hipMemcpyDeviceToHost, ctx->stream));
     if (lw) HIPC(ctx, hipMemcpyAsync(lw, ctx->R.lw, sizeof(double) * n, hipMemcpyDeviceToHost, ctx->stream));
@@ -2253,6 +2281,8 @@
     hipStream_t s = ctx->stream;
     HIPC(ctx, hipMemcpyAsync(w->ybar, agg_bar, sizeof(double) * P * n_het * M, kind, s));
     HIPC(ctx, join_side(ctx));
+    rc = ensure_lot(ctx);
+    if (rc) return rc;
     rc = ensure_adj_seg(ctx);
     if (rc) return rc;
     if (NX > 0) {
@@ -2448,6 +2478,8 @@
     if (rc) return rc;
     *T_out = nullptr;
     if (N == 0) return HANK_OK;
+    rc = ensure_lot(ctx);
+    if (rc) return rc;
     const size_t sz[5] = {P * G * N, G * N, G * N, (size_t)N * P * nbr * NX, (size_t)N * P * NX};
     size_t need = 0, off = 0;
     for (size_t k : sz) carve(need, sizeof(double) * k);
@@ -3140,6 +3172,7 @@
     gf.ss = g.NC >= 16 ? 1 : 0;
     const int RGB = 2, RGF = gf.ss ? 2 : 1;
     const unsigned nbt = (g.nbx + RGB - 1) / RGB, nbf = (gf.nbx + RGF - 1) / RGF + KV, ny = (g.N + g.NC - 1) / g.NC;
+    { const int src = ensure_lot(ctx); if (src) return src; }
     { const int src = ensure_seg(ctx); if (src) return src; }
     { const int src = ensure_lwg(ctx); if (src) return src; }
     HIPC(ctx, join_side(ctx));
@@ -3234,6 +3267,8 @@
         return fail(ctx, HANK_ERR_BAD_ARG, "hank_ss_vjp: n_e=%d needs more LDS per workgroup than the device has", c.n_e);
     if (!ctx->d_adj_sb) HIPC(ctx, ctx->d_adj_sb.alloc((size_t)c.P * c.n_e * ((size_t)c.n_a + 1)));
     HIPC(ctx, join_side(ctx));
+    rc = ensure_lot(ctx);
+    if (rc) return rc;
     rc = ensure_adj_seg(ctx);
     if (rc) return rc;
     if (NX > 0) { rc = ensure_hx_record(ctx); if (rc) return rc; }
diff --git a/julia-newtonraphsonhank_amd/csrc/hank_kernels.h b/julia-newtonraphsonhank_amd/csrc/hank_kernels.h
--- a/julia-newtonraphsonhank_amd/csrc/hank_kernels.h
+++ b/julia-newtonraphsonhank_amd/csrc/hank_kernels.h
@@ -309,7 +309,15 @@
     __shared__ int sh_clo;
     const int col = blockIdx.x;
     if (col >= ncols) return;
-    lottery_body(c, R, col, err, write_seg, use_ib, shlo, &sh_clo, lq);
+    lottery_body<HANK_LOTTERY_LAZY != 0>(c, R, col, err, write_seg, use_ib, shlo, &sh_clo, lq);
+}
+__global__ void __launch_bounds__(256) k_lottery_unpack(Record R, const int4 *__restrict__ lq, const double *__restrict__ iga, int n_a, size_t npt) {
+    const size_t i = (size_t)blockIdx.x * blockDim.x + threadIdx.x;
+    if (i >= npt) return;
+    const int4 q = lq[i];
+    R.lo[i] = q.z;
+    R.lw[i] = __hiloint2double(q.y, q.x);
+    R.ig[i] = (q.w & 1) ? 0.0 : iga[min((unsigned)q.z, (unsigned)(n_a - 1))];
 }
 __global__ void k_iga_build(Consts c, double *iga) {
     const int l = blockIdx.x * blockDim.x + threadIdx.x;
diff --git a/julia-newtonraphsonhank_amd/csrc/hank_xsweep.h b/julia-newtonraphsonhank_amd/csrc/hank_xsweep.h
--- a/julia-newtonraphsonhank_amd/csrc/hank_xsweep.h
+++ b/julia-newtonraphsonhank_amd/csrc/hank_xsweep.h
@@ -226,9 +226,53 @@
 __device__ __forceinline__ void xpublish(XSync *sy, int x, int c, unsigned episode) {
     if ((threadIdx.x & 63) == 0) *reinterpret_cast<volatile unsigned *>(&sy->flag[x][c][0]) = episode;
 }
-__device__ __forceinline__ void xpoll(XSync *sy, int x, int lo, int hi, unsigned need) {
+#if HANK_XPOLL_DEPTH > 1
+__device__ __forceinline__ bool xpoll_block(const unsigned *line, unsigned need) {
+    constexpr int K = HANK_XPOLL_DEPTH;
+    static_assert(K >= 2 && K <= 4, "HANK_XPOLL_DEPTH: 1 .. 4");
+    unsigned done, cnt, t, s0, s1, s2, s3;
+#define XP_TEST(r) "s_waitcnt vmcnt(%[w])\n\tv_sub_u32 %[t], " r ", %[need]\n\tv_cmp_gt_i32 vcc, 0, %[t]\n\ts_cbranch_vccz 2f\n\tglobal_load_dword " r ", %[a], off sc1\n\ts_sleep 1\n\t"
+#define XP_PRIME(r) "global_load_dword " r ", %[a], off sc1\n\ts_sleep 1\n\t"
+#define XP_LOOP_END "s_sub_u32 %[cnt], %[cnt], 1\n\ts_cmp_lg_u32 %[cnt], 0\n\ts_cbranch_scc1 1b\n\ts_mov_b32 %[done], 0\n\ts_branch 3f\n2:\n\ts_mov_b32 %[done], 1\n3:\n\ts_waitcnt vmcnt(0)"
+#define XP_OUT [done] "=&s"(done), [cnt] "=&s"(cnt), [t] "=&v"(t)
+#define XP_IN [a] "v"(line), [need] "v"(need), [w] "n"(K - 1), [n] "n"(64 / K)
+    if constexpr (K == 2)
+        asm volatile(XP_PRIME("%[s0]") XP_PRIME("%[s1]") "s_mov_b32 %[cnt], %[n]\n1:\n\t" XP_TEST("%[s0]") XP_TEST("%[s1]") XP_LOOP_END
+                     : XP_OUT, [s0] "=&v"(s0), [s1] "=&v"(s1) : XP_IN : "vcc", "scc", "memory");
+    else if constexpr (K == 3)
+        asm volatile(XP_PRIME("%[s0]") XP_PRIME("%[s1]") XP_PRIME("%[s2]") "s_mov_b32 %[cnt], %[n]\n1:\n\t" XP_TEST("%[s0]") XP_TEST("%[s1]") XP_TEST("%[s2]") XP_LOOP_END
+                     : XP_OUT, [s0] "=&v"(s0), [s1] "=&v"(s1), [s2] "=&v"(s2) : XP_IN : "vcc", "scc", "memory");
+    else
+        asm volatile(XP_PRIME("%[s0]") XP_PRIME("%[s1]") XP_PRIME("%[s2]") XP_PRIME("%[s3]") "s_mov_b32 %[cnt], %[n]\n1:\n\t" XP_TEST("%[s0]") XP_TEST("%[s1]") XP_TEST("%[s2]")
+                     XP_TEST("%[s3]") XP_LOOP_END
+                     : XP_OUT, [s0] "=&v"(s0), [s1] "=&v"(s1), [s2] "=&v"(s2), [s3] "=&v"(s3) : XP_IN : "vcc", "scc", "memory");
+#undef XP_TEST
+#undef XP_PRIME
+#undef XP_LOOP_END
+#undef XP_OUT
+#undef XP_IN
+    (void)t; (void)s0; (void)s1; (void)s2; (void)s3;
+    return done != 0u;
+}
+#endif
+__device__ __forceinline__ void xpoll(XSync *sy, int x, int lo, int hi, unsigned need, bool spare = false) {
     const int lane = threadIdx.x & 63;
     const XDeadline dl;
+#if HANK_XPOLL_DEPTH > 1
+    if (spare) {
+        const bool in = lane >= lo && lane <= hi;
+        const unsigned *line = &sy->flag[x][(in ? lane : lo) & 63][0];
+        const unsigned need_l = in ? need : 0u;
+        for (unsigned spins = 63u;; spins += 64u) {
+            if (xpoll_block(line, need_l)) break;
+            if (dl.expired(spins) || ((spins & 255u) == 255u && xldu(&sy->status[0]) != 0u)) {
+                if (lane == 0) xfail(sy, XERR_TIMEOUT, x, dl.waited_us());
+                break;
+            }
+        }
+        return;
+    }
+#endif
     for (unsigned spins = 0;; spins++) {
         const unsigned f = (lane >= lo && lane <= hi) ? xldu(&sy->flag[x][lane][0]) : need;
         if (__all((int)(f - need) >= 0)) break;
@@ -239,8 +283,8 @@
         __builtin_amdgcn_s_sleep(1);
     }
 }
-__device__ __forceinline__ void xbar_wait(XSync *sy, int x, int c, int members, unsigned episode, bool sync_wave) {
-    if (sync_wave) { xpublish(sy, x, c, episode); xpoll(sy, x, 0, members - 1, episode); }
+__device__ __forceinline__ void xbar_wait(XSync *sy, int x, int c, int members, unsigned episode, bool sync_wave, bool spare = false) {
+    if (sync_wave) { xpublish(sy, x, c, episode); xpoll(sy, x, 0, members - 1, episode, spare); }
     xlds_barrier();
 }
 
@@ -527,7 +571,7 @@
             }
             episode++;
             xbar_arrive(!syncw);
-            xbar_wait(A.sy, x, cW, Sact, episode, sync_duty);
+            xbar_wait(A.sy, x, cW, Sact, episode, sync_duty, syncw);
         }
     }
 }
@@ -665,7 +709,7 @@
     const bool need_vD = anyclo && clo == 0 && __any(own && (sg0 <= 0 && s2 > 0));
     unsigned episode = 1;
     xbar_arrive(!syncw);
-    xbar_wait(A.sy, x, cW, Sact, episode, sync_duty);
+    xbar_wait(A.sy, x, cW, Sact, episode, sync_duty, syncw);
     int cur = 0, it = 0, conv = 0;
     bool vnz = false;
     for (it = 1; it <= A.max_iter; it++) {
@@ -816,7 +860,7 @@
         XSTAMP(0, son, i, 0);
         if (i > 0) {
             const int t = P - i, cur = (i - 1) & 1;
-            if (sync_duty) xpoll(A.sy, x, srcsh[t] & 255, srcsh[t] >> 8, (unsigned)i);
+            if (sync_duty) xpoll(A.sy, x, srcsh[t] & 255, srcsh[t] >> 8, (unsigned)i, syncw);
             xlds_barrier();
             XSTAMP(0, son, i, 1);
             double dV[D];
@@ -843,7 +887,7 @@
             if (!syncw) xtile_store_n<SL, D>(myt, dV);
             XSTAMP(0, son, i, 2);
             XSTAMPV(0, son, i);
-            if (sync_duty) xpoll(A.sy, x, 0, Sact - 1, (unsigned)i);
+            if (sync_duty) xpoll(A.sy, x, 0, Sact - 1, (unsigned)i, syncw);
             xlds_barrier();
             XSTAMP(0, son, i, 3);
         }
@@ -1033,7 +1077,7 @@
             XSTAMP(0, son, i, 4);
             xbar_arrive(!syncw);
             XSTAMP(0, son, i, 5);
-            xbar_wait(A.sy, x, cW, Sact, episode, sync_duty);
+            xbar_wait(A.sy, x, cW, Sact, episode, sync_duty, syncw);
         }
     }
     XSTAMP1(0, son, 11);
@@ -1292,7 +1336,7 @@
             set_g(I0);
             set_g(I1);
         }
-        if (sync_duty) xpoll(A.sy, x, sw & 255, (sw >> 8) & 255, (unsigned)(t + 1));
+        if (sync_duty) xpoll(A.sy, x, sw & 255, (sw >> 8) & 255, (unsigned)(t + 1), syncw);
         xlds_barrier();
         XSTAMP(1, son, t, 1);
         if (sync_duty && t > 0) reduce_agg(t - 1);
@@ -1399,7 +1443,7 @@
         }
         XSTAMP(1, son, t, 3);
         XSTAMPV(1, son, t);
-        if (sync_duty) xpoll(A.sy, x, 0, Sact - 1, (unsigned)(t + 1));
+        if (sync_duty) xpoll(A.sy, x, 0, Sact - 1, (unsigned)(t + 1), syncw);
         xlds_barrier();
         XSTAMP(1, son, t, 4);
         vnz = ((sw >> 16) & 1) != 0;
```
